# adam-kerrigan/pybader

Hardware: AMD Instinct MI355X
Metric: Mvoxels/s neargrid assign+refine on 512^3 grid (higher is better)
Workload: dtype f64; 1 GPU; 512^3 synthetic 8-Gaussian-atom cubic cell (BASELINE config 3), neargrid assign + neargrid edge refinement changed:2, density resident in HBM; method=neargrid, device_driven_slab_step=False, basins=8

## Files before the change

include/bader_hip.h:

```cpp
#ifndef BADER_HIP_H
#define BADER_HIP_H

#include <stdint.h>

#ifdef __cplusplus
extern "C" {
#endif

typedef struct xb_ctx xb_ctx;

enum { XB_OK = 0, XB_E_ARG = -1, XB_E_HIP = -2, XB_E_STATE = -3, XB_E_LIMIT = -4, XB_E_COMM = -5,
       XB_E_SHORT = -6  };

enum { XB_I8 = 1, XB_I16 = 2, XB_I32 = 4, XB_I64 = 8 };

enum { XB_METHOD_ONGRID = 0, XB_METHOD_NEARGRID = 1 };
enum { XB_REFINE_ALL = 0, XB_REFINE_CHANGED = 1 };

const char *xb_last_error(void);
int xb_device_count(void);
int xb_create(int device, xb_ctx **out);
void xb_destroy(xb_ctx *c);
int xb_sync(xb_ctx *c);
void *xb_stream(xb_ctx *c);
// ... 172 lines not shown
int xb_brick_masks(xb_ctx *c, void **dev_ptr, int64_t *n_bricks, int64_t *own_first, int64_t *own_count);
int xb_table_ties(xb_ctx *c, int64_t *has_ties);
int xb_table_finish(xb_ctx *c, const int64_t *seeds, int64_t n_seeds, int64_t any_ties);

void *xb_labels_ptr(xb_ctx *c);
void *xb_known_ptr(xb_ctx *c);
void *xb_density_ptr(xb_ctx *c);
int64_t xb_plane_elems(xb_ctx *c);
int xb_copy_planes(xb_ctx *c, int which , int to_device, void *host, int64_t xa, int64_t xb);
int xb_label_wire(xb_ctx *c, int widen_to, int *wire_out);
int xb_brick_masks_copy(xb_ctx *c, int to_device, int32_t *host, int64_t first, int64_t count);
int xb_set_halo(xb_ctx *c, int64_t halo);

int xb_slab_supported(xb_ctx *c, int nranks, int64_t *ok);
int xb_slab_assign_masks(xb_ctx *c, int rank, int nranks);
int xb_slab_assign_trace(xb_ctx *c);
int xb_slab_assign_finish(xb_ctx *c, int64_t *n_maxima, int64_t *status);
int xb_slab_refine_pass(xb_ctx *c);
int xb_slab_walkers_round(xb_ctx *c, int src, int last);
int xb_slab_walk_layout(xb_ctx *c, int64_t out[5]);
int xb_slab_walk_send(xb_ctx *c, int64_t walkers);
enum {
    XB_XC_EDGES = 0,
    XB_XC_CHANGED = 1,
    XB_XC_ESCAPED = 2,
    XB_XC_TRAVELLING = 3,
    XB_XC_SLOW = 4,
    XB_XC_LOST = 5,
    XB_XC_MINE = 6,
    XB_XC_ROUNDS = 7,
    XB_XC_COUNT = 8
};
int xb_slab_refine_counts(xb_ctx *c, int64_t *local, int64_t *global);
int xb_slab_block(xb_ctx *c, int which, void **dev_ptr, int64_t *bytes_total, int64_t *own_offset, int64_t *own_bytes);
int xb_slab_block_copy(xb_ctx *c, int which, int to_device, void *host, int64_t off, int64_t bytes);
int xb_host_waits(int64_t *n);

enum {
    XB_TIMER_ASSIGN = 0,
    XB_TIMER_OG_MASKS = 1,
    XB_TIMER_EDGE_FIND = 2,
    XB_TIMER_REFINE_TRACE = 3,
    XB_TIMER_MASKS_GROWTH = 4,
    XB_TIMER_BRICK_MASKS = 5,
    XB_TIMER_TRACE = 6,
    XB_TIMER_BRICK_RECORDS = 7,
    XB_TIMER_MOMENTS = 8,
    XB_TIMER_ADJACENCY = 9,
    XB_TIMER_MERGE = 10,
    XB_TIMER_COUNT = 11
};
int xb_kernel_time(xb_ctx *c, int which, double *ms_total, int64_t *launches);
int xb_kernel_time_reset(xb_ctx *c);
int xb_enable_timing(xb_ctx *c, int on);
enum {
    XB_OPT_REGIONS = 1,
    XB_OPT_CROSS_CHECK = 2,
    XB_OPT_DEBUG = 3,
    XB_OPT_EC_GROUPS = 4,
    XB_OPT_EC_QCAP = 5,
    XB_OPT_DROP_TABLE = 6,
    XB_OPT_KILL_LAUNCHES = 17,
    XB_OPT_SELF_EXCHANGE = 19,
    XB_OPT_ASYNC_COMM = 24,
    XB_OPT_WEIGHT_NO_LABELS = 30
};
enum {
    XB_REGIONS_BOXES = 1,
    XB_REGIONS_BRICKS = 2
};
enum { XB_DROP_TABLE_AND_MAXIMA = 2 };
enum {
    XB_CHECK_NO_MIRROR = 1,
    XB_CHECK_GENERIC_WALKER = 2,
    XB_CHECK_FULL_TGRAD = 4,
    XB_CHECK_LIST_DILATE = 8,
    XB_CHECK_WIDE_HALO = 16,
    XB_CHECK_NO_EC_SHARE = 32,
    XB_CHECK_IO_GATHER = 64
};
#define XB_CHECK_BRICK_LOOKUP 128
#define XB_CHECK_VOXEL_SWEEP 256
#define XB_CHECK_GENERIC_RETRACE 512
enum {
    XB_DBG_EC_PASSES = 4,
    XB_DBG_SLAB_STATS = 16,
    XB_DBG_STAGE_WAIT = 32,
    XB_DBG_SHORT_TIERS = 64
};
#define XB_DBG_KEEP_RETRACE_OVERFLOW 128
int xb_set_option(xb_ctx *c, int key, int value);
int xb_host_alloc(int64_t bytes, void **out);
int xb_host_free(void *p);
int xb_memory_stats(xb_ctx *c, int64_t *bytes_total, int64_t *bytes_table, int64_t *bytes_scratch);
int xb_box_stats(xb_ctx *c, int64_t *n_boxes, int64_t *box_voxels);
int xb_brick_labels(xb_ctx *c, int32_t *out, int64_t capacity, int64_t dims[3]);
int xb_slow_path_stats(xb_ctx *c, int64_t *assign_total, int64_t *refine_total);
int xb_deferred_stats(xb_ctx *c, int64_t *refine_total);
int xb_sweep_stats(xb_ctx *c, int64_t *bit_sweeps, int64_t *voxel_sweeps);
int xb_retrace_stats(xb_ctx *c, int64_t *lean_launches, int64_t *generic_launches);
int xb_trace_stats(xb_ctx *c, int64_t *nb_lean_launches, int64_t *lookup_lean_launches, int64_t *generic_launches,
                   int64_t *wide_lean_launches);
int xb_retrace_overflow(xb_ctx *c, int32_t *out, int64_t capacity, int64_t *n);
int xb_edge_list(xb_ctx *c, int32_t *out, int64_t capacity, int64_t *edges, int64_t *tiles_listed);
int xb_growth_stats(xb_ctx *c, int64_t *retries, int64_t *kill_launches);

int xb_comm_unique_id(uint8_t id_out[128]);
int xb_comm_init(xb_ctx *c, int rank, int nranks, const uint8_t id_in[128]);
int xb_comm_destroy(xb_ctx *c);
int xb_comm_exchange_planes(xb_ctx *c, int which, int n_send, const int32_t *send_peer, const int64_t *send_xa,
                            const int64_t *send_xb, int n_recv, const int32_t *recv_peer, const int64_t *recv_xa,
                            const int64_t *recv_xb);
int xb_comm_allreduce_i64(xb_ctx *c, int64_t *inout, int64_t n, int op);
int xb_comm_allgather_i64(xb_ctx *c, const int64_t *in, int64_t n, int64_t *out);
int xb_comm_share_brick_masks(xb_ctx *c, const int64_t *first, const int64_t *count);
int xb_comm_allgather_block(xb_ctx *c, int which, const int64_t *first, const int64_t *count);
int xb_comm_allreduce_block(xb_ctx *c);
int xb_comm_info(xb_ctx *c, int64_t out[4]);
int xb_comm_stats(xb_ctx *c, int64_t *bytes_sent);

#ifdef __cplusplus
}
#endif
#endif
```

pybader_amd/_lib.py:

```python
import ctypes as C
import threading
import os

import numpy as np

HERE = os.path.dirname(os.path.abspath(__file__))
LIB_PATH = os.environ.get('XB_LIBRARY') or os.path.join(HERE, 'libbader_hip.so')

METHODS = {'ongrid': 0, 'neargrid': 1}
REFINE_MODES = {'all': 0, 'changed': 1}
DTYPE_CODE = {np.dtype(np.int8): 1, np.dtype(np.int16): 2, np.dtype(np.int32): 4, np.dtype(np.int64): 8}
(XB_XC_EDGES, XB_XC_CHANGED, XB_XC_ESCAPED, XB_XC_TRAVELLING, XB_XC_SLOW, XB_XC_LOST, XB_XC_MINE, XB_XC_ROUNDS,
 XB_XC_COUNT) = range(9)
(XB_TIMER_ASSIGN, XB_TIMER_OG_MASKS, XB_TIMER_EDGE_FIND, XB_TIMER_REFINE_TRACE, XB_TIMER_MASKS_GROWTH, XB_TIMER_BRICK_MASKS,
 XB_TIMER_TRACE, XB_TIMER_BRICK_RECORDS, XB_TIMER_MOMENTS, XB_TIMER_ADJACENCY, XB_TIMER_MERGE, XB_TIMER_COUNT) = range(12)
XB_OPT_REGIONS = 1
XB_REGIONS_BOXES, XB_REGIONS_BRICKS = 1, 2
XB_OPT_CROSS_CHECK = 2
(XB_CHECK_NO_MIRROR, XB_CHECK_GENERIC_WALKER, XB_CHECK_FULL_TGRAD, XB_CHECK_LIST_DILATE, XB_CHECK_WIDE_HALO,
 XB_CHECK_NO_EC_SHARE, XB_CHECK_IO_GATHER) = (1, 2, 4, 8, 16, 32, 64)
CROSS_CHECK_BRICK_LOOKUP = 128
CROSS_CHECK_VOXEL_SWEEP = 256
CROSS_CHECK_GENERIC_RETRACE = 512
XB_OPT_DEBUG = 3
XB_DBG_EC_PASSES, XB_DBG_SLAB_STATS, XB_DBG_STAGE_WAIT, XB_DBG_SHORT_TIERS = 4, 16, 32, 64
DEBUG_KEEP_RETRACE_OVERFLOW = 128
XB_OPT_EC_GROUPS = 4
XB_OPT_EC_QCAP = 5
XB_OPT_DROP_TABLE = 6
XB_DROP_TABLE_AND_MAXIMA = 2
XB_OPT_KILL_LAUNCHES = 17
XB_OPT_SELF_EXCHANGE = 19
XB_OPT_ASYNC_COMM = 24
XB_OPT_WEIGHT_NO_LABELS = 30
XB_VORONOI_FULL_SEARCH = 1
XB_VORONOI_CAND_MAX = 512
XB_CRITICAL_FLOOD = 1
(XB_CRITICAL_MAXIMA, XB_CRITICAL_BOND_VOXELS, XB_CRITICAL_BOND_SUM, XB_CRITICAL_RING_VOXELS, XB_CRITICAL_RING_SUM,
 XB_CRITICAL_MINIMA, XB_CRITICAL_COUNTS) = range(7)
XB_CRITICAL_FULL = 0x3fff
XB_CRITICAL_LUT_SIZE = 16384
XB_STENCIL_GATHER = 1
XB_STENCIL_COEFFS = 51
XB_STENCIL_POINT_VALUES = 10
NCI_C = float.fromhex('0x1.8bfd4dd6882cbp+2')
XB_NCI_ATTRACTIVE, XB_NCI_VDW, XB_NCI_REPULSIVE, XB_NCI_CLASSES = range(4)
XB_NCI_HIST_LDS_BINS = 1024
XB_NCI_BINS_MAX = 1 << 24
XB_ISO_GATHER = 1
XB_ISO_TABLE_SIZE = 768
ISO_NCI_RAISED = 100.0
XB_DOMAINS_ABOVE = 0
XB_DOMAINS_BELOW = 1
XB_DOMAINS_NCI = 2
XB_DOMAINS_GLOBAL = 1
XB_DOMAINS_SHARES_LIST = 2
XB_DOMAINS_GATHER = 4
XB_DOMAINS_TIMES = 8
XB_DOMAINS_SHARE_CELLS = 1 << 24
XB_HIRSHFELD_FULL_SEARCH = 1
XB_HIRSHFELD_CAND_MAX = 256
XB_HIRSHFELD_PROMOLECULE, XB_HIRSHFELD_DEFORMATION = 0, 1
XB_ISA_DIRECT = 2
XB_ISA_ITERS_MAX = 64
XB_MBIS_DIRECT = 2
XB_MBIS_KEEP = 4
XB_MBIS_ITERS_MAX = 64
XB_MBIS_SHELLS_MAX = 8
XB_STOCKMOM_DIRECT = 2

_vp, _i64, _dbl, _int = C.c_void_p, C.c_int64, C.c_double, C.c_int
_pi64, _pdbl = C.POINTER(C.c_int64), C.POINTER(C.c_double)
SYMBOLS = {
    'xb_last_error': (C.c_char_p, []),
    'xb_device_count': (_int, []),
    'xb_create': (_int, [_int, C.POINTER(_vp)]),
    'xb_destroy': (None, [_vp]),
    'xb_sync': (_int, [_vp]),
    'xb_stream': (_vp, [_vp]),
    'xb_set_grid': (_int, [_vp, _pi64, _pdbl, _pdbl, _i64, _i64]),
    'xb_upload_density': (_int, [_vp, _vp]),
    'xb_synth_density': (_int, [_vp, _pdbl, _pdbl, _i64, _dbl]),
    'xb_parse_density_text': (_int, [_vp, _vp, _i64, _dbl, _pi64, _pi64]),
    'xb_parse_cube_text': (_int, [_vp, _vp, _i64, _i64, _i64, _int, _dbl, _pi64, _pi64]),
    'xb_download_density': (_int, [_vp, _vp]),
    'xb_format_begin': (_int, [_vp, _vp, _pi64, _int, _dbl, _int, _int, _vp, _i64, _i64, _pi64]),
    'xb_format_host_values': (_int, [_vp, _vp, _vp]),
    'xb_format_set_host_text': (_int, [_vp, _vp, _vp]),
    'xb_format_next': (_int, [_vp, C.POINTER(_vp), _pi64]),
    'xb_format_times': (_int, [_vp, _pdbl, _pdbl]),
    'xb_format_end': (_int, [_vp]),
    'xb_upload_labels': (_int, [_vp, _vp, _int]),
    'xb_download_labels': (_int, [_vp, _vp, _int]),
    'xb_import_density': (_int, [_vp, _vp, _int, _pi64, _vp]),
    'xb_import_labels': (_int, [_vp, _vp, _int, _vp]),
    'xb_export_labels': (_int, [_vp, _vp, _int, _vp]),
    'xb_export_volume': (_int, [_vp, _i64, _vp, _int, _vp]),
    'xb_device_alloc': (_int, [_int, _i64, C.POINTER(_vp)]),
    'xb_device_free': (_int, [_vp]),
    'xb_device_read': (_int, [_vp, _vp, _vp, _i64, _vp]),
    'xb_upload_known': (_int, [_vp, _vp]),
    'xb_download_known': (_int, [_vp, _vp]),
    'xb_vacuum_assign': (_int, [_vp, _dbl, _dbl, _pdbl, _pdbl]),
    'xb_assign': (_int, [_vp, _int, _pi64]),
    'xb_get_maxima': (_int, [_vp, _vp, _i64]),
    'xb_assign_trace': (_int, [_vp, _int, _pi64]),
# ... 24 lines not shown
    'xb_adjacency_release': (_int, [_vp]),
    'xb_merge_basins': (_int, [_vp, _vp, _int, _i64, _vp, _dbl, _i64, _pi64, _pi64, C.POINTER(_int)]),
    'xb_merge_fetch': (_int, [_vp, _vp, _vp, _vp, _i64]),
    'xb_merge_release': (_int, [_vp]),
    'xb_weight_sum': (_int, [_vp, _pdbl, _dbl, _vp, _pi64]),
    'xb_weight_sum_device': (_int, [_vp, _pdbl, _dbl, _vp, _int, _pi64, _vp, _pi64]),
    'xb_weight_fetch': (_int, [_vp, _vp, _vp, _vp, _i64]),
    'xb_weight_stats': (_int, [_vp, _pi64]),
    'xb_weight_release': (_int, [_vp]),
    'xb_voronoi_assign': (_int, [_vp, _pdbl, _pdbl, _i64, _dbl, _int, _pi64]),
    'xb_critical_lut': (_int, [_vp]),
    'xb_critical_points': (_int, [_vp, _dbl, _int, _pi64, _pi64]),
    'xb_critical_fetch': (_int, [_vp, _vp, _vp, _vp, _vp, _i64]),
    'xb_critical_bonds': (_int, [_vp, _i64, _pi64, _pi64]),
    'xb_critical_bonds_fetch': (_int, [_vp, _vp, _vp, _vp, _vp, _vp, _i64]),
    'xb_critical_release': (_int, [_vp]),
    'xb_stencil_coeffs': (_int, [_pdbl, _i64, _i64, _i64, _pdbl]),
    'xb_laplacian_field': (_int, [_vp, _pdbl, _int, _vp, _vp]),
    'xb_laplacian_sum': (_int, [_vp, _pdbl, _i64, _dbl, _int, _pdbl, _pdbl, _pdbl]),
    'xb_stencil_points': (_int, [_vp, _pdbl, _vp, _i64, _vp]),
    'xb_nci_field': (_int, [_vp, _pdbl, _int, _vp, _vp, _vp, _vp]),
    'xb_nci_sum': (_int, [_vp, _pdbl, _i64, _dbl, _dbl, _dbl, _dbl, _int, _pi64, _pdbl, _pdbl]),
    'xb_nci_hist': (_int, [_vp, _pdbl, _pdbl, _i64, _pdbl, _i64, _int, _pi64]),
    'xb_isosurface_table': (_int, [_vp]),
    'xb_isosurface': (_int, [_vp, _vp, _vp, _pdbl, _dbl, _i64, _int, _pi64]),
    'xb_isosurface_fetch': (_int, [_vp, _int, _vp, _vp, _vp, _vp, _vp, _i64, _i64, _pdbl, _pdbl, _i64]),
    'xb_isosurface_release': (_int, [_vp]),
    'xb_isosurface_nci_mask': (_int, [_vp, _vp, _dbl]),
    'xb_regions_label': (_int, [_vp, _int, _vp, _dbl, _pdbl, _dbl, _dbl, _int, _pi64]),
    'xb_regions_sums': (_int, [_vp, _dbl, _dbl, _pi64, _pi64, _pi64, _pdbl, _pdbl, _pi64, _pdbl, _pdbl, _i64]),
    'xb_regions_shares': (_int, [_vp, _i64, _int, _pi64]),
    'xb_regions_shares_fetch': (_int, [_vp, _vp, _vp, _pi64, _i64]),
    'xb_regions_fetch_map': (_int, [_vp, _int, _vp]),
    'xb_regions_times': (_int, [_vp, _pdbl]),
    'xb_regions_release': (_int, [_vp]),
    'xb_stream_wait': (_int, [_vp, _vp]),
    'xb_device_write': (_int, [_vp, _vp, _vp, _i64]),
    'xb_hirshfeld_images': (_int, [_pdbl, _pdbl, _vp, _i64, _pdbl, _i64, _pi64, _vp, _i64]),
    'xb_hirshfeld_setup': (_int, [_vp, _pdbl, _pdbl, _vp, _i64, _pdbl, _pdbl, _i64, _i64]),
    'xb_hirshfeld_release': (_int, [_vp]),
    'xb_hirshfeld_sum': (_int, [_vp, _dbl, _int, _pdbl, _pdbl, _pdbl, _pi64]),
    'xb_hirshfeld_field': (_int, [_vp, _int, _int, _vp, _vp]),
    'xb_isa_setup': (_int, [_vp, _pdbl, _pdbl, _i64, _pdbl, _i64, _pdbl, _dbl, _pi64]),
    'xb_isa_iterate': (_int, [_vp, _i64, _int, _pi64, _pi64]),
    'xb_isa_tables': (_int, [_vp, _pdbl, _pi64]),
    'xb_isa_load': (_int, [_vp, _pdbl]),
    'xb_isa_rho_bound': (_int, [_vp, _pdbl]),
    'xb_mbis_setup': (_int, [_vp, _pdbl, _pdbl, _i64, _pdbl, _vp, _pdbl, _i64, _i64, _pdbl, _pdbl, _dbl, _dbl, _pi64]),
    'xb_mbis_iterate': (_int, [_vp, _i64, _int, _pi64, _pi64, _pi64, _pi64]),
    'xb_mbis_params': (_int, [_vp, _pdbl, _pdbl, _pi64]),
    'xb_mbis_load': (_int, [_vp, _pdbl, _pdbl]),
    'xb_mbis_field': (_int, [_vp, _int, _int, _vp, _vp]),
    'xb_stockholder_moments': (_int, [_vp, _dbl, _int, _pi64, _pi64, _pi64]),
    'xb_volume_assign': (_int, [_vp, _vp, _i64]),
    'xb_atom_assign': (_int, [_vp, _i64, _vp, _i64, _vp, _vp, _vp]),
    'xb_surface_distance': (_int, [_vp, _vp, _vp, _i64, _vp, _pi64]),
    'xb_volume_mask': (_int, [_vp, _i64, _vp]),
    'xb_label_sum': (_int, [_vp, _i64, _pdbl, _pi64]),
    'xb_set_table_window': (_int, [_vp, _i64]),
    'xb_table_build': (_int, [_vp, _pi64]),
    'xb_table_local_seeds': (_int, [_vp, _vp, _i64]),
    'xb_brick_masks': (_int, [_vp, C.POINTER(_vp), _pi64, _pi64, _pi64]),
    'xb_table_ties': (_int, [_vp, _pi64]),
    'xb_table_finish': (_int, [_vp, _vp, _i64, _i64]),
    'xb_labels_ptr': (_vp, [_vp]),
    'xb_known_ptr': (_vp, [_vp]),
    'xb_density_ptr': (_vp, [_vp]),
    'xb_plane_elems': (_i64, [_vp]),
    'xb_copy_planes': (_int, [_vp, _int, _int, _vp, _i64, _i64]),
    'xb_label_wire': (_int, [_vp, _int, _vp]),
    'xb_host_alloc': (_int, [_i64, _vp]),
    'xb_host_free': (_int, [_vp]),
    'xb_brick_masks_copy': (_int, [_vp, _int, _vp, _i64, _i64]),
    'xb_set_halo': (_int, [_vp, _i64]),
    'xb_kernel_time': (_int, [_vp, _int, _pdbl, _pi64]),
    'xb_kernel_time_reset': (_int, [_vp]),
    'xb_enable_timing': (_int, [_vp, _int]),
    'xb_set_option': (_int, [_vp, _int, _int]),
    'xb_box_stats': (_int, [_vp, _pi64, _pi64]),
    'xb_brick_labels': (_int, [_vp, _vp, _i64, _pi64]),
    'xb_slow_path_stats': (_int, [_vp, _pi64, _pi64]),
    'xb_deferred_stats': (_int, [_vp, _pi64]),
    'xb_sweep_stats': (_int, [_vp, _pi64, _pi64]),
    'xb_edge_list': (_int, [_vp, _vp, _i64, _pi64, _pi64]),
    'xb_retrace_stats': (_int, [_vp, _pi64, _pi64]),
    'xb_trace_stats': (_int, [_vp, _pi64, _pi64, _pi64, _pi64]),
    'xb_axis_limits': (_int, [_vp, _pi64, _pi64]),
    'xb_retrace_overflow': (_int, [_vp, _vp, _i64, _pi64]),
    'xb_growth_stats': (_int, [_vp, _pi64, _pi64]),
    'xb_comm_unique_id': (_int, [_vp]),
    'xb_comm_init': (_int, [_vp, _int, _int, _vp]),
    'xb_comm_destroy': (_int, [_vp]),
    'xb_comm_exchange_planes': (_int, [_vp, _int, _int, _vp, _pi64, _pi64, _int, _vp, _pi64, _pi64]),
    'xb_comm_allreduce_i64': (_int, [_vp, _pi64, C.c_int64, _int]),
    'xb_comm_allgather_i64': (_int, [_vp, _pi64, C.c_int64, _pi64]),
    'xb_comm_share_brick_masks': (_int, [_vp, _pi64, _pi64]),
    'xb_comm_allgather_block': (_int, [_vp, _int, _pi64, _pi64]),
    'xb_comm_allreduce_block': (_int, [_vp]),
    'xb_slab_supported': (_int, [_vp, _int, _pi64]),
    'xb_slab_assign_masks': (_int, [_vp, _int, _int]),
    'xb_slab_assign_trace': (_int, [_vp]),
    'xb_slab_assign_finish': (_int, [_vp, _pi64, _pi64]),
    'xb_slab_refine_pass': (_int, [_vp]),
    'xb_slab_walkers_round': (_int, [_vp, _int, _int]),
    'xb_slab_walk_layout': (_int, [_vp, _pi64]),
    'xb_slab_walk_send': (_int, [_vp, _i64]),
    'xb_slab_refine_counts': (_int, [_vp, _pi64, _pi64]),
    'xb_slab_block': (_int, [_vp, _int, C.POINTER(_vp), _pi64, _pi64, _pi64]),
    'xb_slab_block_copy': (_int, [_vp, _int, _int, _vp, _i64, _i64]),
    'xb_host_waits': (_int, [_pi64]),
    'xb_comm_stats': (_int, [_vp, _pi64]),
    'xb_comm_info': (_int, [_vp, _pi64]),
    'xb_memory_stats': (_int, [_vp, _pi64, _pi64, _pi64]),
}

_lib = None


class BaderHipError(RuntimeError):
    code = None


XB_E_ARG = -1
XB_E_STATE = -3
XB_E_LIMIT = -4
XB_E_SHORT = -6


def load():
    global _lib
    if _lib is None:
        if not os.path.exists(LIB_PATH):
            raise BaderHipError(f"{LIB_PATH} is missing: build it with `python -m pybader_amd.build` "
                                "(hipcc, gfx950); pybader_amd has no CPU fallback")
        lib = C.CDLL(LIB_PATH)
        for name, (res, args) in SYMBOLS.items():
            fn = getattr(lib, name)
            fn.restype = res
            fn.argtypes = args
        _lib = lib
    return _lib


_POOL_KEEP = 4
_POOL_MAX_BYTES = 4 << 30


class _PinnedBuf:
    __slots__ = ('ptr', 'nbytes', '__weakref__')

    def __init__(self, ptr, nbytes):
        self.ptr, self.nbytes = ptr, nbytes

    @property
    def __array_interface__(self):
        return {'shape': (self.nbytes,), 'typestr': '|u1', 'data': (self.ptr, False), 'version': 3}


_pool = {}
_pool_bytes = 0
_pool_lock = threading.Lock()


def _host_free(ptr):
    if _lib is not None:
        _lib.xb_host_free(C.c_void_p(ptr))
# ... 1008 lines not shown
    def slab_block(self, which):
        p, a, b, d = _vp(), C.c_int64(0), C.c_int64(0), C.c_int64(0)
        check(self.lib.xb_slab_block(self.h, int(which), C.byref(p), C.byref(a), C.byref(b), C.byref(d)))
        return int(p.value or 0), int(a.value), int(b.value), int(d.value)

    def slab_block_copy(self, which, host, off, to_device):
        assert host.dtype == np.uint8 and host.flags.c_contiguous
        check(self.lib.xb_slab_block_copy(self.h, int(which), 1 if to_device else 0, _ptr(host), int(off), host.nbytes))

    def comm_allgather_block(self, which, first, count):
        f, n = np.array(first, np.int64), np.array(count, np.int64)
        check(self.lib.xb_comm_allgather_block(self.h, int(which), f.ctypes.data_as(_pi64), n.ctypes.data_as(_pi64)))

    def comm_allreduce_block(self):
        check(self.lib.xb_comm_allreduce_block(self.h))

    def host_waits(self):
        a = C.c_int64(0)
        check(self.lib.xb_host_waits(C.byref(a)))
        return int(a.value)

    def memory_stats(self):
        a, b, d = C.c_int64(0), C.c_int64(0), C.c_int64(0)
        check(self.lib.xb_memory_stats(self.h, C.byref(a), C.byref(b), C.byref(d)))
        return int(a.value), int(b.value), int(d.value)

    def comm_info(self):
        out = (C.c_int64 * 4)()
        check(self.lib.xb_comm_info(self.h, out))
        return {'nccl_comm_count': int(out[0]), 'nccl_user_rank': int(out[1]), 'nccl_device': int(out[2]), 'rccl_version': int(out[3])}

    def comm_bytes_sent(self):
        n = C.c_int64(0)
        check(self.lib.xb_comm_stats(self.h, C.byref(n)))
        return int(n.value)

    def enable_timing(self, on=True, only=None):
        mask = int(bool(on)) if only is None else sum(2 << int(k) for k in only)
        check(self.lib.xb_enable_timing(self.h, mask))

    def kernel_time(self, which):
        ms, n = C.c_double(), C.c_int64()
        check(self.lib.xb_kernel_time(self.h, int(which), C.byref(ms), C.byref(n)))
        return ms.value, n.value

    def kernel_time_reset(self):
        check(self.lib.xb_kernel_time_reset(self.h))

    def set_option(self, key, value):
        check(self.lib.xb_set_option(self.h, int(key), int(value)))

    def box_stats(self):
        a, b = C.c_int64(), C.c_int64()
        check(self.lib.xb_box_stats(self.h, C.byref(a), C.byref(b)))
        return a.value, b.value

    def brick_labels(self):
        dims = (C.c_int64 * 3)()
        check(self.lib.xb_brick_labels(self.h, None, 0, dims))
        out = np.zeros(tuple(int(d) for d in dims), np.int32)
        check(self.lib.xb_brick_labels(self.h, _ptr(out), out.size, dims))
        return out

    def slow_path_stats(self):
        a, b = C.c_int64(), C.c_int64()
        check(self.lib.xb_slow_path_stats(self.h, C.byref(a), C.byref(b)))
        return a.value, b.value

    def growth_stats(self):
        a, b = C.c_int64(), C.c_int64()
        check(self.lib.xb_growth_stats(self.h, C.byref(a), C.byref(b)))
        return a.value, b.value

    def deferred_stats(self):
        a = C.c_int64()
        check(self.lib.xb_deferred_stats(self.h, C.byref(a)))
        return a.value

    def sweep_stats(self):
        a, b = C.c_int64(), C.c_int64()
        check(self.lib.xb_sweep_stats(self.h, C.byref(a), C.byref(b)))
        return a.value, b.value

    def retrace_stats(self):
        a, b = C.c_int64(), C.c_int64()
        check(self.lib.xb_retrace_stats(self.h, C.byref(a), C.byref(b)))
        return a.value, b.value

    def trace_stats(self):
        a, b, g = C.c_int64(), C.c_int64(), C.c_int64()
        check(self.lib.xb_trace_stats(self.h, C.byref(a), C.byref(b), C.byref(g), None))
        return a.value, b.value, g.value

    def trace_offset_stats(self):
        a, b, w = C.c_int64(), C.c_int64(), C.c_int64()
        check(self.lib.xb_trace_stats(self.h, C.byref(a), C.byref(b), None, C.byref(w)))
        return a.value + b.value - w.value, w.value

    def axis_limits(self):
        a, b = C.c_int64(), C.c_int64()
        check(self.lib.xb_axis_limits(self.h, C.byref(a), C.byref(b)))
        return a.value, b.value

    def retrace_overflow(self):
        n = C.c_int64()
        check(self.lib.xb_retrace_overflow(self.h, None, 0, C.byref(n)))
        out = np.zeros(n.value, np.int32)
        if n.value:
            check(self.lib.xb_retrace_overflow(self.h, _ptr(out), out.size, C.byref(n)))
        return out

    def edge_list(self):
        n, t = C.c_int64(), C.c_int64()
        check(self.lib.xb_edge_list(self.h, None, 0, C.byref(n), C.byref(t)))
        out = np.zeros(n.value, np.int32)
        if n.value:
            check(self.lib.xb_edge_list(self.h, _ptr(out), out.size, C.byref(n), C.byref(t)))
        return out, t.value

    def sync(self):
        check(self.lib.xb_sync(self.h))


def critical_lut():
    out = np.zeros(XB_CRITICAL_LUT_SIZE, np.uint8)
    check(load().xb_critical_lut(_ptr(out)))
    return out


def isosurface_table():
    out = np.zeros(XB_ISO_TABLE_SIZE, np.uint8)
    check(load().xb_isosurface_table(_ptr(out)))
    return out.reshape(6, 16, 8)


def hirshfeld_images(lattice, atoms_cart, species, r_cut):
    lat, at = _f64(lattice).reshape(9), _f64(atoms_cart).reshape(-1, 3)
    sp, rc = np.ascontiguousarray(species, dtype=np.int32).reshape(-1), _f64(r_cut).reshape(-1)
    if sp.shape[0] != at.shape[0]:
        raise ValueError(f'hirshfeld_images: {sp.shape[0]} species for {at.shape[0]} atoms')
    lib, m = load(), C.c_int64()
    args = (lat.ctypes.data_as(_pdbl), at.ctypes.data_as(_pdbl), _ptr(sp), at.shape[0], rc.ctypes.data_as(_pdbl), rc.shape[0])
    check(lib.xb_hirshfeld_images(*args, C.byref(m), None, 0))
    out = np.zeros((int(m.value), 4), np.int32)
    check(lib.xb_hirshfeld_images(*args, C.byref(m), _ptr(out), out.shape[0]))
    return out


def stencil_coeffs(lattice, shape):
    lat = _f64(lattice).reshape(9)
    out = np.zeros(XB_STENCIL_COEFFS, np.float64)
    nx, ny, nz = (int(s) for s in shape)
    check(load().xb_stencil_coeffs(lat.ctypes.data_as(_pdbl), nx, ny, nz, out.ctypes.data_as(_pdbl)))
    return out[:9].reshape(3, 3), out[9:15], out[15:].reshape(6, 6)


def atom_assign(bader_max_cart, atoms_cart, lattice):
    lib = load()
    bm, at, lat = _f64(bader_max_cart).reshape(-1, 3), _f64(atoms_cart).reshape(-1, 3), _f64(lattice).reshape(9)
    a, d = np.zeros(bm.shape[0], np.int64), np.zeros(bm.shape[0], np.float64)
    check(lib.xb_atom_assign(_ptr(bm), bm.shape[0], _ptr(at), at.shape[0], _ptr(lat), _ptr(a), _ptr(d)))
    return a, d


_default_ctx = {}

# ... 10 lines not shown
```

pybader_amd/csrc/bader_hip.hip:

```cpp
#include "bader_kernels.h"
#include "../../include/bader_hip.h"
#include "ctx_state.h"
#include "ctx_buffers.h"

#include <algorithm>
#include <cmath>
#include <cstdarg>
#include <cstdio>
#include <cstring>
#include <locale.h>
#include <mutex>
#include <numeric>
#include <string>
#include <thread>
#include <vector>

static thread_local long long xb_waits = 0;
static inline hipError_t xb_counted_sync(hipStream_t s) { xb_waits++; return (hipStreamSynchronize)(s); }
#define hipStreamSynchronize(s) xb_counted_sync(s)

#include "k_common.h"
#include "k_masks.h"
#include "k_fused.h"
#include "k_trace.h"
#include "k_ongrid.h"
#include "k_edges.h"
#include "k_sums.h"
#include "k_text.h"
#include "k_format.h"
#include "k_interop.h"
#include "k_weight.h"
#include "k_cell.h"
#include "k_moments.h"
#include "k_adjacency.h"
#include "k_merge.h"
#include "k_voronoi.h"
#include "k_critical.h"
#include "k_stencil.h"
#include "k_nci.h"
#include "k_hirshfeld.h"
#include "k_isa.h"
#include "k_mbis.h"
#include "k_stockmom.h"
#include "k_isosurface.h"
#include "k_regions.h"

static thread_local std::string g_err;
static int fail(int code, const char *fmt, ...) {
    char buf[512];
    va_list ap;
    va_start(ap, fmt);
    vsnprintf(buf, sizeof buf, fmt, ap);
    va_end(ap);
    g_err = buf;
    return code;
}
#define XB_BIG_CHUNK ((size_t)16 << 20)
#define HIPCHK(x)                                                                                   \
    do {                                                                                            \
        hipError_t e_ = (x);                                                                        \
        if (e_ != hipSuccess) return fail(XB_E_HIP, "%s:%d %s: %s", __FILE__, __LINE__, #x, hipGetErrorString(e_)); \
    } while (0)

struct TimedKernel {
    std::vector<std::pair<hipEvent_t, hipEvent_t>> pending;
    double ms = 0.;
    long long launches = 0;
};

namespace xbcomm { struct State; }
struct xb_ctx : CtxState, CtxBuffers {
    int device = 0;
    xbcomm::State *comm = nullptr;
    struct FmtState *fmt = nullptr;
    hipStream_t stream = nullptr;
    Grid g{};
    bool has_grid = false;
    long long N = 0;
    int halo = 0;
    double *rho = nullptr;
    GradRec *grad = nullptr;
    long long grad_cap = 0;
    long long list_cap = 0;
    int *ec_buf = nullptr;
    long long ec_buf_cap = 0;
    double *dist_dev = nullptr;
    int *boxbuf = nullptr;
    int *box_max_tab = nullptr;
    int n_boxes = 0;
    long long box_voxels = 0;
    struct Options {
        int boxes = 1, bricks = 1;
        int mirror = 1;
        int lean = 1;
        int mask_diag = 1;
        int tile_dilate = 1;
        int narrow_halo = 1;
        int ec_share = 1;
        int nb_bits = 1;
        int bit_sweep = 1;
        int lean_retrace = 1;
        int io_tiled = 1;
        int dbg = 0;
        int ec_groups = 256;
        int ec_qcap = EC_Q;
        int self_exchange = 0;
        int async_comm = 0;
        bool weight_no_labels = false;
    } opt;
    int *ec_share = nullptr;
    std::vector<int64_t> esc_starts, esc_offsets, esc_vox;
    unsigned long long *ec_pend = nullptr;
    int8_t *ec_pflag = nullptr;
    std::vector<int8_t> esc_complete;
    double vac_tol = 0.;
    bool regions_pending = false;
    bool buni_halo_safe = false;
    bool regions_neargrid = false;
    int n_walk = 0;
    int *walk = nullptr;
    int table_margin = -1;
    bool table_prebuilt = false;
    int table_stage = 0;
    std::vector<int> window_seeds;
    bool window_ties = true;
    bool slab_sparse = false;
    int ec_local_n = 0;
    int walk_n_out = 0;
    void *walk_out_dev = nullptr;
    std::vector<int64_t> walk_host, res_host;
    int walk_n_res = 0;
    void *walk_in = nullptr, *walk_out2 = nullptr, *walk_res = nullptr;
    long long walk_cap = 0;
    long long stat_deferred = 0;
    long long stat_bit_sweeps = 0, stat_voxel_sweeps = 0;
    long long stat_ovf_assign = 0, stat_ovf_refine = 0;
    long long stat_lean_retraces = 0, stat_generic_retraces = 0;
    long long stat_nb_traces = 0, stat_lookup_traces = 0, stat_generic_traces = 0;
    long long stat_wide_traces = 0;
    int max_grid[3] = {0, 0, 0};
    std::vector<int> dbg_retrace_ovf;
    int *bres_last = nullptr;
    int *blab = nullptr;
    int nbk[3] = {0, 0, 0};
    bool brick_max_blanket = false;
    int grad_cover = 0;
    unsigned char *brick_rec = nullptr;
    unsigned long long *nb_tab = nullptr;
    void *xbuf = nullptr;
    int slab_rank = 0, slab_nranks = 0, slab_stage = 0;
    void *wbuf[2] = {nullptr, nullptr};
    void *wk_in = nullptr;
    int wbuf_ranks = 0, walk_last = -1, walk_round = 0, wcap = 0;
    int walk_send = 0;
    int grow_kill_launches = 6;
    long long stat_grow_retries = 0;
    bool defer_wait = false;
    bool pending_assign = false;
    int64_t pending_n_maxima = 0;
    int grad_rule = 0;
    int *labels = nullptr;
    int8_t *known = nullptr;
    int *first = nullptr;
    int *list = nullptr;
    int8_t *st = nullptr;
    void *stage = nullptr;
    size_t stage_bytes = 0;
    int *max_list = nullptr;
    int *max_aux = nullptr;
    int max_cap = 0;
    int *ovf_list = nullptr;
    int ovf_cap = 0;
    int *counters = nullptr;
    int *fs = nullptr;
    int *blab_buf = nullptr;
    long long blab_alloc = 0;
    static constexpr int trace_waves = 8192;
    unsigned long long *counters64 = nullptr;
    double *dsum = nullptr;
    int *host_ints = nullptr;
    char *big_pin[2] = {nullptr, nullptr};
    hipEvent_t big_ev[2] = {nullptr, nullptr};
    hipEvent_t io_ev = nullptr;
    char *pin = nullptr;
    size_t pin_bytes = 0;
    std::vector<int> maxima_sorted;
    std::vector<int> local_max, local_first;
    bool first_clean = false;
    int list_n = 0;
    bool tiles_listed = false;
    unsigned timing = 0;
    TimedKernel tk[XB_TIMER_COUNT];
    long long n_alloc = 0;
    bool thin = false;
    long long w_stat[6] = {0, 0, 0, 0, 0, 0};
    bool w_have = false;
    std::vector<int64_t> w_idx;
    std::vector<double> w_charge, w_volume;
    bool aj_have = false;
    int aj_dirs = 0;
    std::vector<int32_t> aj_a, aj_b;
    std::vector<int64_t> aj_facets, aj_sfacet;
    std::vector<double> aj_saddle;
    bool mg_have = false;
    std::vector<int32_t> mg_root, mg_round;
    std::vector<double> mg_pers;
    size_t cp_n = 0, cp_bond_voxels = 0;
    bool cb_have = false;
    std::vector<unsigned long long> cp_rec;
    std::vector<int32_t> cb_a, cb_b;
    std::vector<int64_t> cb_saddles, cb_voxel;
    std::vector<double> cb_rho;
    size_t hs_acc = 0;
    bool hs_have = false;
    int64_t hs_n = 0;
    int hs_cus = 0;
    HsGeom hs_geom{};
    bool hs_isa = false;
    size_t isa_x = 0, isa_pairs0 = 0;
    int isa_e = 0, isa_cur = 0;
    double isa_bound = 0.;
    bool hs_mbis = false;
    size_t mbis_x = 0;
    int mbis_M = 0, mbis_MS = 0, mbis_cur = 0, mbis_e[4] = {0, 0, 0, 0};
    int64_t mbis_J = 0, mbis_KE = 0;
// ... 64 lines not shown
        if (std::memcmp(&a, &b, sizeof a) != 0) return false;
        s.dsym[idx] = a;
    }
    return true;
}

static void mirror_prefilter(const Grid &g, int &mirror, double &mu_scale) {
    mirror = 0;
    double dmin = 0.;
    bool first = true;
    for (int i = 0; i < 27; i++)
        if (i != 0) { dmin = first ? g.dist[i] : std::min(dmin, g.dist[i]); first = false; }
    if (!(dmin > 0.) || !std::isfinite(dmin)) { mu_scale = 0.; return; }
    for (int ax = 0; ax < 3; ax++) {
        bool ok = true;
        for (int u = 0; u < 3 && ok; u++)
            for (int v = 0; v < 3 && ok; v++) {
                int ip[3], im[3];
                ip[ax] = 1; im[ax] = 2;
                ip[(ax + 1) % 3] = im[(ax + 1) % 3] = u;
                ip[(ax + 2) % 3] = im[(ax + 2) % 3] = v;
                const double a = g.dist[ip[0] * 9 + ip[1] * 3 + ip[2]], b = g.dist[im[0] * 9 + im[1] * 3 + im[2]];
                ok = std::memcmp(&a, &b, sizeof a) == 0;
            }
        if (ok) mirror |= 1 << ax;
    }
    mu_scale = std::ldexp(1. + 1. / dmin, -48);
}

struct ScopedTimer {
    xb_ctx *c;
    int which;
    hipEvent_t a = nullptr, b = nullptr;
    ScopedTimer(xb_ctx *c_, int w) : c(c_), which(w) {
        if ((c->timing >> which) & 1u) {
            hipEventCreate(&a);
            hipEventCreate(&b);
            hipEventRecord(a, c->stream);
        }
    }
    ~ScopedTimer() {
        if ((c->timing >> which) & 1u) {
            hipEventRecord(b, c->stream);
            c->tk[which].pending.push_back({a, b});
        }
    }
};

extern "C" {

const char *xb_last_error(void) { return g_err.c_str(); }

#include "host_context.h"
#include "host_stages.h"
#include "host_format.h"
#include "host_assign.h"
#include "host_refine.h"
#include "host_sums.h"
#include "host_slab_table.h"
#include "host_interop.h"
#include "host_weight.h"
#include "host_cell.h"
#include "host_moments.h"
#include "host_adjacency.h"
#include "host_merge.h"
#include "host_voronoi.h"
#include "host_critical.h"
#include "host_stencil.h"
#include "host_nci.h"
#include "host_hirshfeld.h"
#include "host_isa.h"
#include "host_mbis.h"
#include "host_stockmom.h"
#include "host_isosurface.h"
#include "host_regions.h"
#include "host_analyses.h"

int xb_set_option(xb_ctx *c, int key, int value) {
    if (!c) return fail(XB_E_ARG, "null ctx");
    bool ok = true;
    switch (key) {
    case XB_OPT_REGIONS: c->opt.boxes = (value & XB_REGIONS_BOXES) != 0; c->opt.bricks = (value & XB_REGIONS_BRICKS) != 0; break;
    case XB_OPT_CROSS_CHECK:
        if (!(ok = value >= 0 && value < 2 * XB_CHECK_GENERIC_RETRACE)) break;
        c->opt.mirror = !(value & XB_CHECK_NO_MIRROR);
        c->opt.lean = !(value & XB_CHECK_GENERIC_WALKER);
        c->opt.mask_diag = !(value & XB_CHECK_FULL_TGRAD);
        c->opt.tile_dilate = !(value & XB_CHECK_LIST_DILATE);
        c->opt.narrow_halo = !(value & XB_CHECK_WIDE_HALO);
        c->opt.ec_share = !(value & XB_CHECK_NO_EC_SHARE);
        c->opt.io_tiled = !(value & XB_CHECK_IO_GATHER);
        c->opt.nb_bits = !(value & XB_CHECK_BRICK_LOOKUP);
        c->opt.bit_sweep = !(value & XB_CHECK_VOXEL_SWEEP);
        c->opt.lean_retrace = !(value & XB_CHECK_GENERIC_RETRACE);
        break;
    case XB_OPT_DEBUG: c->opt.dbg = value; break;
    case XB_OPT_EC_GROUPS: if ((ok = value >= 1 && value <= 4096)) c->opt.ec_groups = value; break;
    case XB_OPT_EC_QCAP: if ((ok = value >= 2 && value <= EC_Q)) c->opt.ec_qcap = value; break;
    case XB_OPT_DROP_TABLE: if (value == XB_DROP_TABLE_AND_MAXIMA) drop_table_and_maxima(*c); else drop_table(*c); break;
    case XB_OPT_KILL_LAUNCHES: if ((ok = value >= 1)) c->grow_kill_launches = value; break;
    case XB_OPT_SELF_EXCHANGE: c->opt.self_exchange = value != 0; break;
    case XB_OPT_ASYNC_COMM: c->opt.async_comm = value != 0; break;
    case XB_OPT_WEIGHT_NO_LABELS: c->opt.weight_no_labels = value != 0; break;
    default: ok = false;
    }
    if (!ok) return fail(XB_E_ARG, "xb_set_option: unknown key %d", key);
    return XB_OK;
}
int xb_growth_stats(xb_ctx *c, int64_t *retries, int64_t *kill_launches) {
    if (!c) return fail(XB_E_ARG, "null ctx");
    if (retries) *retries = c->stat_grow_retries;
    if (kill_launches) *kill_launches = c->grow_kill_launches;
    return XB_OK;
}
int xb_deferred_stats(xb_ctx *c, int64_t *refine_total) {
    if (!c) return fail(XB_E_ARG, "null ctx");
    if (refine_total) *refine_total = c->stat_deferred;
    return XB_OK;
}
int xb_sweep_stats(xb_ctx *c, int64_t *bit_sweeps, int64_t *voxel_sweeps) {
    if (!c) return fail(XB_E_ARG, "null ctx");
    if (bit_sweeps) *bit_sweeps = c->stat_bit_sweeps;
    if (voxel_sweeps) *voxel_sweeps = c->stat_voxel_sweeps;
    return XB_OK;
}
int xb_retrace_stats(xb_ctx *c, int64_t *lean_launches, int64_t *generic_launches) {
    if (!c) return fail(XB_E_ARG, "null ctx");
    if (lean_launches) *lean_launches = c->stat_lean_retraces;
    if (generic_launches) *generic_launches = c->stat_generic_retraces;
    return XB_OK;
}
int xb_trace_stats(xb_ctx *c, int64_t *nb_lean_launches, int64_t *lookup_lean_launches, int64_t *generic_launches, int64_t *wide_lean_launches) {
    if (!c) return fail(XB_E_ARG, "null ctx");
    if (wide_lean_launches) *wide_lean_launches = c->stat_wide_traces;
    if (nb_lean_launches) *nb_lean_launches = c->stat_nb_traces;
    if (lookup_lean_launches) *lookup_lean_launches = c->stat_lookup_traces;
    if (generic_launches) *generic_launches = c->stat_generic_traces;
    return XB_OK;
}
int xb_retrace_overflow(xb_ctx *c, int32_t *out, int64_t capacity, int64_t *n) {
    if (!c || !n || capacity < 0 || (capacity > 0 && !out)) return fail(XB_E_ARG, "xb_retrace_overflow: null ctx / count, or a capacity without a buffer");
    *n = (int64_t)c->dbg_retrace_ovf.size();
    if (capacity >= *n) {
        std::copy(c->dbg_retrace_ovf.begin(), c->dbg_retrace_ovf.end(), out);
        c->dbg_retrace_ovf.clear();
    }
    return XB_OK;
}
int xb_slow_path_stats(xb_ctx *c, int64_t *assign_total, int64_t *refine_total) {
    if (!c) return fail(XB_E_ARG, "null ctx");
    if (assign_total) *assign_total = c->stat_ovf_assign;
    if (refine_total) *refine_total = c->stat_ovf_refine;
    return XB_OK;
}
int xb_memory_stats(xb_ctx *c, int64_t *bytes_total, int64_t *bytes_table, int64_t *bytes_scratch) {
    if (!c || !c->has_grid) return fail(XB_E_STATE, "xb_memory_stats: no grid");
    const long long N = c->N;
    const long long table = c->grad_cap * (long long)sizeof(GradRec);
    const long long scratch = c->list_cap * 4 + (long long)c->stage_bytes + c->ec_buf_cap * 4 + (c->ec_pend ? 8 * N + 16 : 0) +
                              (long long)buf_counted_bytes(*c) ;
    const long long fixed = 8 * N  + 4 * N  + (N + 16)  + 4 * N  + N  +
                            2LL * c->max_cap * 4 + (long long)c->ovf_cap * 4 + c->blab_alloc * 13 + (long long)c->walk_cap * 3 * 80 +
                            (1 << 22) ;
    if (bytes_total) *bytes_total = fixed + table + scratch;
    if (bytes_table) *bytes_table = table;
    if (bytes_scratch) *bytes_scratch = scratch;
    return XB_OK;
}
int xb_box_stats(xb_ctx *c, int64_t *n_boxes, int64_t *box_voxels) {
    if (!c) return fail(XB_E_ARG, "null ctx");
    if (n_boxes) *n_boxes = c->n_boxes;
    if (box_voxels) *box_voxels = c->box_voxels;
    return XB_OK;
}
int xb_brick_labels(xb_ctx *c, int32_t *out, int64_t capacity, int64_t dims[3]) {
    if (!c || !c->has_grid) return fail(XB_E_STATE, "xb_brick_labels: no grid");
    if (!c->blab) return fail(XB_E_STATE, "xb_brick_labels: no trapping regions on this context (no neargrid assignment yet)");
    const int64_t nbr = (int64_t)c->nbk[0] * c->nbk[1] * c->nbk[2];
    if (dims) { dims[0] = c->nbk[0]; dims[1] = c->nbk[1]; dims[2] = c->nbk[2]; }
    if (!out) return XB_OK;
    if (capacity < nbr) return fail(XB_E_ARG, "xb_brick_labels: capacity too small");
    HIPCHK(hipSetDevice(c->device));
    HIPCHK(hipMemcpyAsync(out, c->blab, nbr * sizeof(int), hipMemcpyDeviceToHost, c->stream));
    HIPCHK(hipStreamSynchronize(c->stream));
    return XB_OK;
}
#ifdef XB_DEBUG_COUNT
int xb_debug_steps(xb_ctx *c, int on, signed char *host_out) {
    static signed char *buf = nullptr;
    if (host_out && buf) {
        if (hipMemcpy(host_out, buf, (size_t)c->N, hipMemcpyDeviceToHost) != hipSuccess) return XB_E_HIP;
    }
    if (on && !buf && hipMalloc(&buf, (size_t)c->N) != hipSuccess) return XB_E_HIP;
    if (on && hipMemset(buf, 0, (size_t)c->N) != hipSuccess) return XB_E_HIP;
    signed char *p = on ? buf : nullptr;
    return hipMemcpyToSymbol(HIP_SYMBOL(xb_dbg_steps), &p, sizeof p) == hipSuccess ? XB_OK : XB_E_HIP;
}
int xb_debug_counts(unsigned long long *out, int reset) {
    hipDeviceSynchronize();
    if (out && hipMemcpyFromSymbol(out, HIP_SYMBOL(xb_dbg), sizeof(unsigned long long) * 65536) != hipSuccess) return XB_E_HIP;
    if (reset) {
        static unsigned long long z[65536];
        if (hipMemcpyToSymbol(HIP_SYMBOL(xb_dbg), z, sizeof z) != hipSuccess) return XB_E_HIP;
    }
    return XB_OK;
}
// ... 42 lines not shown
```

pybader_amd/csrc/host_assign.h:

```cpp

static GridL light(const Grid &g);

static int ensure_brick_bytes(xb_ctx *c, int nbr) {
    if (c->blab_alloc < nbr) {
        hipFree(c->blab_buf); c->blab_buf = nullptr; c->blab_alloc = 0; c->brick_rec = nullptr; c->nb_tab = nullptr; c->brick_max_valid = false;
        if (c->grad_cover) { c->grad_cover = 0; drop_table(*c); }
        const size_t rec_bytes = ((size_t)nbr + 16 + 7) & ~(size_t)7;
        HIPCHK(hipMalloc(&c->blab_buf, (size_t)nbr * sizeof(int) + rec_bytes + (size_t)nbr * sizeof(unsigned long long)));
        c->blab_alloc = nbr;
        c->brick_rec = reinterpret_cast<unsigned char *>(c->blab_buf + nbr);
        c->nb_tab = reinterpret_cast<unsigned long long *>(c->brick_rec + rec_bytes);
    }
    return XB_OK;
}

static int ensure_grad(xb_ctx *c, bool force, bool boxes, bool main_rule) {
    if (int rc = need_grad(c)) return rc;
    c->g.main_ties = main_rule ? 1 : 0;
    if (c->grad_valid && !force && (c->grad_rule == 2 || c->grad_rule == (main_rule ? 1 : 0))) return XB_OK;
    const Grid &g = c->g;
    if (c->grad_valid && !force && !boxes && c->grad_cover == 1 && c->brick_rec) {
        const int nb1r = (g.ny + BRK - 1) / BRK, nb2r = (g.nz + BRK - 1) / BRK, nbr = ((g.nx + BRK - 1) / BRK) * nb1r * nb2r;
        ScopedTimer t(c, XB_TIMER_MASKS_GROWTH);
        launch_brick_records(c, nullptr, nullptr, nbr, nb1r, nb2r);
        HIPCHK(hipGetLastError());
        c->grad_rule = main_rule ? 1 : 0;
        return XB_OK;
    }
    if (!force && !boxes && !table_windowed(c) && g.x0 == 0 && g.x1 == g.nx && g.nx >= 16 && g.ny >= 16 && g.nz >= 16) {
        const int nb0 = (g.nx + BRK - 1) / BRK, nb1 = (g.ny + BRK - 1) / BRK, nb2 = (g.nz + BRK - 1) / BRK, nbr = nb0 * nb1 * nb2;
        if (int rc = ensure_brick_bytes(c, nbr)) return rc;
        ScopedTimer t(c, XB_TIMER_MASKS_GROWTH);
        int *buni = reinterpret_cast<int *>(c->st);
        if (!c->buni_valid) k_label_uniform_list<<<4096, TPB, 0, c->stream>>>(light(g), c->labels, nb1, nb2, nullptr, nbr, nullptr, nullptr, buni, 0, nbr);
        c->buni_valid = true;
        k_buni3<<<(nbr + 255) / 256, 256, 0, c->stream>>>(nb0, nb1, nb2, buni, buni + nbr);
        k_flag_mixed_bricks<<<(nbr + 255) / 256, 256, 0, c->stream>>>(nbr, buni + nbr, c->brick_rec);
        launch_brick_records(c, nullptr, nullptr, nbr, nb1, nb2);
        HIPCHK(hipGetLastError());
        c->grad_valid = true;
        c->grad_cover = 1;
        c->brick_max_blanket = true;
        c->grad_rule = main_rule ? 1 : 0;
        c->regions_labels = false;
        c->blab = nullptr;
        c->table_stage = 0;
        return XB_OK;
    }
    {
        const int nb0 = (g.nx + BRK - 1) / BRK, nb1 = (g.ny + BRK - 1) / BRK, nb2 = (g.nz + BRK - 1) / BRK, nbr = nb0 * nb1 * nb2;
        if (int rc = ensure_brick_bytes(c, nbr)) return rc;
        ScopedTimer t(c, XB_TIMER_MASKS_GROWTH);
        ScopedTimer t_masks(c, XB_TIMER_BRICK_MASKS);
        const int wb0 = table_windowed(c) ? g.wx0 / BRK : 0, wnb = table_windowed(c) ? g.wlen / BRK : nb0;
        k_flag_window_bricks<<<(nbr + 255) / 256, 256, 0, c->stream>>>(nb0, nb1 * nb2, wb0, wnb, (unsigned char)3, c->brick_rec);
        launch_brick_records(c, nullptr, nullptr, nbr, nb1, nb2);
        HIPCHK(hipGetLastError());
    }
    c->grad_valid = true;
    c->grad_cover = 1;
    c->brick_max_blanket = true;
    c->grad_rule = main_rule ? 1 : 0;
    c->window_ties = true;
    c->n_boxes = 0;
    c->box_voxels = 0;
    c->blab = nullptr;
    c->regions_labels = false;
    c->window_seeds.clear();
    c->table_stage = 2;
    (void)boxes;
    return XB_OK;
}

static int upload_pinned(xb_ctx *c, void *dst, const void *src, size_t bytes, size_t slot = 0) {
    if (!bytes) return XB_OK;
    if (slot + bytes > c->pin_bytes) {
        HIPCHK(hipStreamSynchronize(c->stream));
        const size_t want = std::max<size_t>(2 * (slot + bytes), 1 << 20);
        char *p = nullptr;
        HIPCHK(hipHostMalloc(&p, want));
        if (c->pin && slot) memcpy(p, c->pin, slot);
        hipHostFree(c->pin);
        c->pin = p; c->pin_bytes = want;
    }
    memcpy(c->pin + slot, src, bytes);
    HIPCHK(hipMemcpyAsync(dst, c->pin + slot, bytes, hipMemcpyHostToDevice, c->stream));
    return XB_OK;
}
static int download_pinned(xb_ctx *c, void *dst, const void *src_dev, size_t bytes) {
    if (!bytes) return XB_OK;
    if (bytes > c->pin_bytes) {
        HIPCHK(hipStreamSynchronize(c->stream));
        hipHostFree(c->pin); c->pin = nullptr; c->pin_bytes = 0;
        const size_t want = std::max<size_t>(2 * bytes, 1 << 20);
        HIPCHK(hipHostMalloc(&c->pin, want));
        c->pin_bytes = want;
    }
    HIPCHK(hipMemcpyAsync(c->pin, src_dev, bytes, hipMemcpyDeviceToHost, c->stream));
    HIPCHK(hipStreamSynchronize(c->stream));
    memcpy(dst, c->pin, bytes);
    return XB_OK;
}

#define XB_MID_K 32
static int run_slow(xb_ctx *c, int n, int refine, int *max_count = nullptr, int *changed = nullptr, int *escaped = nullptr, const int *list_in = nullptr,
                    const int *n_dev = nullptr, bool stage_free = false) {
    if (!max_count) max_count = c->counters + CT_N_MAX;
    if (!changed) changed = c->counters + CT_CHANGED;
    if (!escaped) escaped = c->counters + CT_ESCAPED;
    if (n <= 0) return XB_OK;
    const size_t budget = (size_t)128 << 20;
    const int tiers[3] = {(c->opt.dbg & XB_DBG_SHORT_TIERS) ? 3 : 64, (c->opt.dbg & XB_DBG_SHORT_TIERS) ? 5 : 2048, (c->opt.dbg & XB_DBG_SHORT_TIERS) ? 8 : 1 << 15};
    const bool blind = (size_t)n * tiers[1] <= budget;
    const size_t have = std::max<size_t>(std::min<size_t>(budget, (size_t)n * tiers[0]), blind ? (size_t)n * tiers[1] : 0) + (size_t)(1 << 15) * 64;
    const size_t n_lists = 2 * (size_t)n + 8;
    DevBuf<int> path_buf, lists_buf;
    int *path = nullptr, *lists = nullptr;
// ... 170 lines not shown
                max_count_dev = c->counters + CT_N_MAX;
            }
            if (int rc = run_slow(c, novf, 0)) return rc;
        }
        c->g.main_ties = 0;
    } else if (method == XB_METHOD_ONGRID) {
        c->zero_outside[0] = -1;
        c->blab = nullptr;
        c->n_boxes = 0;
        c->box_voxels = 0;
        {
            ScopedTimer t(c, XB_TIMER_OG_MASKS);
            const int small = small_grid(g);
            const int nbr = ((g.nx + BRK - 1) / BRK) * ((g.ny + BRK - 1) / BRK) * ((g.nz + BRK - 1) / BRK);
            if (3LL * nbr > c->list_cap) return fail(XB_E_LIMIT, "xb_assign: scratch too small for the brick arrays of the pointer pass");
            dim3 grid((g.nz + GT_Z - 1) / GT_Z, (g.ny + GT_Y - 1) / GT_Y, (g.nx + GT_X - 1) / GT_X);
            int *bm = c->list, *bmv = c->list + nbr, *bpt = c->list + 2 * nbr;
            GridS gs;
            if (sym_grid(g, gs)) k_og_masks<GridS, true><<<grid, TPB, 0, c->stream>>>(gs, c->rho, c->labels, small, c->has_vacuum ? 1 : 0, bm, bmv, bpt);
            else k_og_masks<Grid, true><<<grid, TPB, 0, c->stream>>>(g, c->rho, c->labels, small, c->has_vacuum ? 1 : 0, bm, bmv, bpt);
        }
        HIPCHK(hipGetLastError());
        box_max = c->boxbuf + BB_REGMAX;
        for (int it = 0; it < 64; it++) {
            HIPCHK(hipMemsetAsync(c->counters + CT_OG_MOVED, 0, sizeof(int), c->stream));
            k_og_jump<<<nblocks(c->N), TPB, 0, c->stream>>>(g, c->labels, c->counters + CT_OG_MOVED);
            HIPCHK(hipGetLastError());
            int nd = 0;
            if (int rc = read_counter(c, CT_OG_MOVED, &nd)) return rc;
            if (!nd) break;
            if (it == 63) return fail(XB_E_LIMIT, "ongrid pointer jumping did not converge");
        }
        k_note_roots<<<nblocks(own), TPB, 0, c->stream>>>(g, c->labels, c->first, c->max_list, c->counters + CT_N_MAX, c->max_cap);
        HIPCHK(hipGetLastError());
    } else
        return fail(XB_E_ARG, "xb_assign: unknown method %d", method);
    int nmax = 0;
    HIPCHK(hipMemcpyAsync(c->host_ints, max_count_dev, sizeof(int), hipMemcpyDeviceToHost, c->stream));
    HIPCHK(hipStreamSynchronize(c->stream));
    nmax = c->host_ints[0];
    if (nmax > c->max_cap) return fail(XB_E_LIMIT, "%d maxima exceed the table capacity %d", nmax, c->max_cap);
    c->local_max.resize(nmax);
    c->local_first.resize(nmax);
    if (nmax) {
        k_gather_first<<<(nmax + 255) / 256, 256, 0, c->stream>>>(c->first, c->max_list, nmax, c->max_aux);
        HIPCHK(hipGetLastError());
        if (int rc = download_pinned(c, c->local_max.data(), c->max_list, nmax * sizeof(int))) return rc;
        if (int rc = download_pinned(c, c->local_first.data(), c->max_aux, nmax * sizeof(int))) return rc;
    }
    if (n_local) *n_local = nmax;
    return XB_OK;
}

int xb_assign_local_table(xb_ctx *c, int64_t *max_idx, int64_t *first_idx, int64_t capacity) {
    NEED_GRID("xb_assign_local_table");
    if ((int64_t)c->local_max.size() > capacity) return fail(XB_E_ARG, "xb_assign_local_table: capacity too small");
    for (size_t i = 0; i < c->local_max.size(); i++) { max_idx[i] = c->local_max[i]; first_idx[i] = c->local_first[i]; }
    return XB_OK;
}

int xb_assign_finish(xb_ctx *c, const int64_t *max_idx_sorted, int64_t n_global) {
    NEED_GRID("xb_assign_finish");
    if (n_global > c->max_cap) return fail(XB_E_LIMIT, "xb_assign_finish: too many maxima");
    c->maxima_sorted.resize(n_global);
    for (int64_t i = 0; i < n_global; i++) c->maxima_sorted[i] = (int)max_idx_sorted[i];
    c->label_wire = label_wire_for(n_global);
    const Grid &g = c->g;
    if (n_global) {
        if (int rc = upload_pinned(c, c->max_aux, c->maxima_sorted.data(), n_global * sizeof(int))) return rc;
        k_set_rank<<<(unsigned)((n_global + 255) / 256), 256, 0, c->stream>>>(c->first, c->max_aux, (int)n_global);
        HIPCHK(hipGetLastError());
    }
    drop_label_marks(*c);
    const bool regions = c->regions_pending && c->blab;
    int buni = BUNI_NONE;
    if (regions && g.x1 - g.x0 == g.nx)
        buni = BUNI_SCAN;
    else if (regions && !c->has_vacuum && g.nx % 8 == 0 && g.ny % 8 == 0 && g.nz % 8 == 0 && g.x0 % 8 == 0 && g.x1 % 8 == 0)
        buni = BUNI_MIXED;
    launch_relabel(c, nullptr, (int)n_global, regions, c->box_max_tab ? c->box_max_tab : c->boxbuf + BB_REGMAX, buni, nullptr);
    HIPCHK(hipGetLastError());
    if (buni != BUNI_NONE) {
        c->buni_valid = true;
        c->buni_halo_safe = buni == BUNI_MIXED;
    }
    c->regions_labels = regions && !c->has_vacuum && c->regions_neargrid;
    c->regions_pending = false;
    HIPCHK(hipStreamSynchronize(c->stream));
    c->first_clean = true;
    return XB_OK;
}


static bool fused_ok(const xb_ctx *c) {
    const Grid &g = c->g;
    return c->opt.boxes && c->opt.bricks && g.x0 == 0 && g.x1 == g.nx && !table_windowed(c) &&
           g.nx >= 16 && g.ny >= 16 && g.nz >= 16;
}
static int assign_neargrid_tail(xb_ctx *c, int64_t *n_maxima);

static int fused_numbering_launch(xb_ctx *c) {
    k_number_maxima<<<1, 1024, 0, c->stream>>>(c->fs, c->first, c->max_list, c->max_cap, c->max_aux, c->fs + FS_TOTAL);
    launch_relabel(c, c->fs, 0, c->regions_pending, c->box_max_tab, BUNI_SCAN, c->bres_last);
    HIPCHK(hipGetLastError());
    return XB_OK;
}
static int number_maxima_big(xb_ctx *c, int nmax) {
    const long long n_words = (c->N + 31) / 32, n_blocks = (n_words + 1023) / 1024;
    const size_t need = (size_t)(2 * n_words + n_blocks) * sizeof(int);
    DevBuf<int> own;
    int *scratch = (int *)c->stage;
    if (!c->stage || c->stage_bytes < need) {
        HIPCHK(own.alloc((size_t)(2 * n_words + n_blocks)));
        scratch = own.p;
    }
    unsigned *bits = reinterpret_cast<unsigned *>(scratch);
    int *wprefix = scratch + n_words, *bsum = scratch + 2 * n_words;
    HIPCHK(hipMemsetAsync(bits, 0, (size_t)n_words * sizeof(int), c->stream));
    k_rank_mark<<<(nmax + 255) / 256, 256, 0, c->stream>>>(c->first, c->max_list, nmax, bits);
    k_rank_scan<<<(unsigned)n_blocks, 1024, 0, c->stream>>>(bits, (int)n_words, wprefix, bsum);
    k_rank_blocks<<<1, 1024, 0, c->stream>>>(bsum, (int)n_blocks);
    k_rank_assign<<<(nmax + 255) / 256, 256, 0, c->stream>>>(c->first, c->max_list, nmax, bits, wprefix, bsum, c->max_aux, c->fs);
    HIPCHK(hipGetLastError());
    launch_relabel(c, c->fs, 0, c->regions_pending, c->box_max_tab, BUNI_SCAN, c->bres_last);
    HIPCHK(hipGetLastError());
    c->maxima_sorted.resize(nmax);
    HIPCHK(hipMemcpyAsync(c->maxima_sorted.data(), c->max_aux, (size_t)nmax * sizeof(int), hipMemcpyDeviceToHost, c->stream));
    HIPCHK(hipStreamSynchronize(c->stream));
    return XB_OK;
}

static int assign_neargrid_fused(xb_ctx *c, int64_t *n_maxima) {
    if (int rc = need_grad(c)) return rc;
    Grid &g = c->g;
    const int nb0 = (g.nx + BRK - 1) / BRK, nb1 = (g.ny + BRK - 1) / BRK, nb2 = (g.nz + BRK - 1) / BRK, nbr = nb0 * nb1 * nb2;
    const bool part = g.nx % BRK || g.ny % BRK || g.nz % BRK;
    if (int rc = ensure_brick_bytes(c, nbr)) return rc;
    int *fs = c->fs;
    int *seed = c->list, *bmask = c->list + nbr, *buf0 = c->list + 2 * nbr, *buf1 = c->list + 3 * nbr, *walk = c->list + 4 * nbr;
    int *box_max = c->boxbuf + BB_REGMAX, *box_first = c->boxbuf + BB_REGFIRST;
    int *bmaxv = walk;
    int *bpot = c->list + 5 * nbr;
    int *bres = nullptr;
    c->box_max_tab = box_max;
    auto stage_done = [&](const char *what) {
        if (c->opt.dbg & XB_DBG_STAGE_WAIT) {
            const hipError_t e = (hipStreamSynchronize)(c->stream);
            int h16[16] = {0};
            (void)hipMemcpy(h16, fs, sizeof h16, hipMemcpyDeviceToHost);
            fprintf(stderr, "[assign] %s: %s  seeds %d regions %d certain %d walk %d maxima %d ovf %d err %d\n", what, hipGetErrorString(e), h16[FS_N_SEEDS],
                    h16[FS_N_BOXES], h16[FS_N_CERTAIN], h16[FS_N_WALK], h16[FS_N_MAX], h16[FS_N_OVF], h16[FS_ERR]);
            fflush(stderr);
        }
    };
    if (int rc = begin_assignment(c, fs, FS_TOTAL, true)) return rc;
    g.main_ties = 1;
    const GridL gl = light(g);
    {
        ScopedTimer t_growth(c, XB_TIMER_MASKS_GROWTH);
        {
            ScopedTimer t_masks(c, XB_TIMER_BRICK_MASKS);
            launch_brick_masks(c, part, true, bmask, bmaxv, bpot);
        }
        stage_done("brick masks");
        c->grad_valid = true;
        c->grad_rule = 1;
        c->grad_cover = 1;
        launch_region_growth(c, nb0, nb1, nb2, bmask, bmaxv, bpot, seed, buf0, buf1, box_max, box_first, true);
        HIPCHK(hipGetLastError());
        stage_done("region growth");
    }
    c->blab = c->blab_buf;
    c->regions_neargrid = true;
    c->walk = walk;
    c->nbk[0] = nb0; c->nbk[1] = nb1; c->nbk[2] = nb2;
    const long long own = c->N;
    {
        ScopedTimer t_assign(c, XB_TIMER_ASSIGN);
        {
            const bool vac = c->has_vacuum && c->vac_by_tol;
            launch_walk_list(c, nb0, nb1, nb2, walk, vac ? bpot : nullptr, c->vac_tol);
        }
        {
            ScopedTimer t_records(c, XB_TIMER_BRICK_RECORDS);
            launch_brick_records(c, walk, fs + FS_N_WALK, nbr, nb1, nb2);
        }
        stage_done("walk list + records");
        if (c->has_vacuum)
            k_fill_certain<<<nblocks(own), TPB, 0, c->stream>>>(gl, c->blab, nb1, nb2, box_max, c->labels, c->first, c->max_list,
                                                                fs + FS_N_MAX, c->max_cap, fs + FS_GROW_RETRY);
        else {
            k_note_regions<<<1, XB_BOXES_MAX, 0, c->stream>>>(gl, nb1, nb2, fs, box_first, box_max, c->first, c->max_list, fs + FS_N_MAX, c->max_cap);
            c->regions_pending = true;
        }
        {
            ScopedTimer t_trace(c, XB_TIMER_TRACE);
            int *bres_buf = c->has_vacuum ? nullptr : c->list + 6 * nbr;
            if (launch_persistent_trace(c, true, part, box_max, walk, c->has_vacuum ? 1 : 0, bres_buf)) bres = bres_buf;
        }
        HIPCHK(hipGetLastError());
        stage_done("trace");
    }
    c->bres_last = bres;
    if (int rc = fused_numbering_launch(c)) return rc;
    stage_done("numbering + relabel");
    HIPCHK(hipMemcpyAsync(c->host_ints, fs, (FS_TOTAL + XB_SORT_MAX) * sizeof(int), hipMemcpyDeviceToHost, c->stream));
    if (c->defer_wait) {
        g.main_ties = 0;
        c->grad_rule = 2;
        c->regions_pending = false;
        c->buni_valid = !c->has_vacuum;
        c->regions_labels = !c->has_vacuum;
        c->pending_assign = true;
        return XB_OK;
    }
    HIPCHK(hipStreamSynchronize(c->stream));
    return assign_neargrid_tail(c, n_maxima);
}

static int assign_neargrid_tail(xb_ctx *c, int64_t *n_maxima) {
    Grid &g = c->g;
    int *fs = c->fs;
    const int nb1 = c->nbk[1], nb2 = c->nbk[2];
    int *walk = c->walk, *box_max = c->box_max_tab;
    const int *h = c->host_ints;
    g.main_ties = 0;
    const GridL gl = light(g);
    if (h[FS_GROW_RETRY]) {
        c->grow_kill_launches = 1 << 20;
        c->stat_grow_retries++;
        drop_table(*c);
        return assign_neargrid_fused(c, n_maxima);
    }
    if (h[FS_TIES] == 0) c->grad_rule = 2;
    c->n_boxes = h[FS_N_BOXES];
    c->box_voxels = (long long)h[FS_N_CERTAIN] * BRK * BRK * BRK;
    c->n_walk = h[FS_N_WALK];
    const int novf = h[FS_N_OVF];
    int nmax = h[FS_N_MAX];
    if (nmax > c->max_cap) return fail(XB_E_LIMIT, "%d maxima exceed the table capacity %d", nmax, c->max_cap);
    c->stat_ovf_assign += novf;
    const int *sorted = h[FS_SORT_OK] && novf == 0 ? h + FS_TOTAL : nullptr;
    if (novf > 0) {
        g.main_ties = 1;
        const GridL glt = light(g);
        const int maxsteps = trace_maxsteps(g);
        int *list2 = (int *)c->stage;
        const int cap2 = (int)std::min<size_t>(c->stage_bytes / sizeof(int), 0x7fffffffu);
        auto two_tiers = [&](int n_listed) -> int {
            c->host_ints[HI_UPLOAD] = n_listed;
            HIPCHK(hipMemcpyAsync(c->counters + CT_MID_LISTED, c->host_ints + HI_UPLOAD, sizeof(int), hipMemcpyHostToDevice, c->stream));
            HIPCHK(hipMemsetAsync(c->counters + CT_MID_LEFT, 0, sizeof(int), c->stream));
            k_ng_trace_list<XB_MID_K><<<512, TPB, 0, c->stream>>>(glt, c->grad, box_max, c->blab, nb1, nb2, c->ovf_list, c->counters + CT_MID_LISTED, c->labels, c->first,
                                                          c->max_list, fs + FS_N_MAX, c->max_cap, list2, c->counters + CT_MID_LEFT, cap2, maxsteps, c->rho, c->dist_dev,
                                                          c->has_vacuum ? 1 : 0);
            HIPCHK(hipGetLastError());
            if (c->opt.dbg & XB_DBG_EC_PASSES) {
                int m2 = 0;
                if (int rc2 = read_counter(c, CT_MID_LEFT, &m2)) return rc2;
                fprintf(stderr, "[assign] %d walkers listed, %d left for the exact slow kernel after the %d-voxel window\n", n_listed, m2, XB_MID_K);
            }
            if (n_listed > cap2) return fail(XB_E_LIMIT, "%d walkers for the exact slow path exceed its list (%d)", n_listed, cap2);
            return run_slow(c, n_listed, 0, fs + FS_N_MAX, nullptr, nullptr, list2, c->counters + CT_MID_LEFT, true);
        };
        int rc = two_tiers(std::min(novf, c->ovf_cap));
        for (int left = novf - c->ovf_cap; !rc && left > 0;) {
            HIPCHK(hipMemsetAsync(c->counters + CT_N_OVF, 0, sizeof(int), c->stream));
            k_list_unfinished<<<4096, TPB, 0, c->stream>>>(gl, walk, fs + FS_N_WALK, nb1, nb2, c->labels, c->ovf_list, c->counters + CT_N_OVF, c->ovf_cap);
            HIPCHK(hipGetLastError());
            int m = 0;
            if ((rc = read_counter(c, CT_N_OVF, &m))) break;
            if (m == 0) break;
            rc = two_tiers(std::min(m, c->ovf_cap));
            left = m - c->ovf_cap;
        }
        g.main_ties = 0;
        if (rc) return rc;
        HIPCHK(hipMemsetAsync(fs + FS_N_OVF, 0, sizeof(int), c->stream));
        if (int rc2 = fused_numbering_launch(c)) return rc2;
        HIPCHK(hipMemcpyAsync(c->host_ints, fs, (FS_TOTAL + XB_SORT_MAX) * sizeof(int), hipMemcpyDeviceToHost, c->stream));
        HIPCHK(hipStreamSynchronize(c->stream));
        nmax = h[FS_N_MAX];
        if (nmax > c->max_cap) return fail(XB_E_LIMIT, "%d maxima exceed the table capacity %d", nmax, c->max_cap);
        if (h[FS_SORT_OK]) sorted = h + FS_TOTAL;
    }
    if (!sorted) {
        if (int rc = number_maxima_big(c, nmax)) return rc;
    }
    numbering_done(c, sorted, nmax, n_maxima);
    c->buni_valid = !c->has_vacuum;
    c->regions_labels = !c->has_vacuum;
    return XB_OK;
}


static bool assign_neargrid_complete(xb_ctx *c, int64_t *n_maxima) {
    c->pending_assign = false;
    const int *h = c->host_ints;
    const int nmax = h[FS_N_MAX];
    if (h[FS_GROW_RETRY] || h[FS_TIES] != 0 || h[FS_N_OVF] != 0 || !h[FS_SORT_OK] || nmax > c->max_cap || nmax > XB_SORT_MAX) return false;
    c->n_boxes = h[FS_N_BOXES];
    c->box_voxels = (long long)h[FS_N_CERTAIN] * BRK * BRK * BRK;
    c->n_walk = h[FS_N_WALK];
    numbering_done(c, h + FS_TOTAL, nmax, n_maxima);
    return true;
}

static int assign_ongrid_fused(xb_ctx *c, int64_t *n_maxima) {
    Grid &g = c->g;
    const int nb0 = (g.nx + BRK - 1) / BRK, nb1 = (g.ny + BRK - 1) / BRK, nb2 = (g.nz + BRK - 1) / BRK, nbr = nb0 * nb1 * nb2;
    const bool part = g.nx % BRK || g.ny % BRK || g.nz % BRK;
    if (int rc = ensure_brick_bytes(c, nbr)) return rc;
    int *fs = c->fs;
    int *seed = c->list, *bmask = c->list + nbr, *buf0 = c->list + 2 * nbr, *buf1 = c->list + 3 * nbr, *walk = c->list + 4 * nbr;
    int *bmaxv = walk, *bpot = c->list + 5 * nbr;
    int *box_max = c->boxbuf + BB_REGMAX, *box_first = c->boxbuf + BB_REGFIRST;
    c->box_max_tab = box_max;
    if (int rc = begin_assignment(c, fs, FS_TOTAL, true)) return rc;
    c->zero_outside[0] = -1;
    const GridL gl = light(g);
    {
        ScopedTimer t(c, XB_TIMER_OG_MASKS);
        const int small = small_grid(g);
        dim3 grid((g.nz + GT_Z - 1) / GT_Z, (g.ny + GT_Y - 1) / GT_Y, (g.nx + GT_X - 1) / GT_X);
        GridS gs;
        if (sym_grid(g, gs)) {
            if (part) k_og_masks<GridS, true><<<grid, TPB, 0, c->stream>>>(gs, c->rho, c->labels, small, 0, bmask, bmaxv, bpot);
            else k_og_masks<GridS, false><<<grid, TPB, 0, c->stream>>>(gs, c->rho, c->labels, small, 0, bmask, bmaxv, bpot);
        } else {
            if (part) k_og_masks<Grid, true><<<grid, TPB, 0, c->stream>>>(g, c->rho, c->labels, small, 0, bmask, bmaxv, bpot);
            else k_og_masks<Grid, false><<<grid, TPB, 0, c->stream>>>(g, c->rho, c->labels, small, 0, bmask, bmaxv, bpot);
        }
    }
    {
        ScopedTimer t_growth(c, XB_TIMER_MASKS_GROWTH);
        launch_region_growth(c, nb0, nb1, nb2, bmask, bmaxv, bpot, seed, buf0, buf1, box_max, box_first, true);
        HIPCHK(hipGetLastError());
    }
    drop_table(*c);
    c->grad_cover = 0;
    c->brick_max_valid = true;
    c->brick_max_blanket = false;
    c->blab = c->blab_buf;
    c->regions_neargrid = false;
    c->walk = walk;
    c->bres_last = nullptr;
    c->nbk[0] = nb0; c->nbk[1] = nb1; c->nbk[2] = nb2;
    {
        ScopedTimer t_assign(c, XB_TIMER_ASSIGN);
        launch_walk_list(c, nb0, nb1, nb2, walk, nullptr, 0.);
        k_note_regions<<<1, XB_BOXES_MAX, 0, c->stream>>>(gl, nb1, nb2, fs, box_first, box_max, c->first, c->max_list, fs + FS_N_MAX, c->max_cap);
        c->regions_pending = true;
        k_og_walk_dev<<<16384, XB_WAVE, 0, c->stream>>>(gl, box_max, c->blab, nb1, nb2, walk, fs, c->labels, c->first, c->max_list, c->max_cap,
                                                        1 << 22);
        HIPCHK(hipGetLastError());
    }
    if (int rc = fused_numbering_launch(c)) return rc;
    HIPCHK(hipMemcpyAsync(c->host_ints, fs, (FS_TOTAL + XB_SORT_MAX) * sizeof(int), hipMemcpyDeviceToHost, c->stream));
    HIPCHK(hipStreamSynchronize(c->stream));
    const int *h = c->host_ints;
    if (h[FS_GROW_RETRY]) {
        c->grow_kill_launches = 1 << 20;
        c->stat_grow_retries++;
        return assign_ongrid_fused(c, n_maxima);
    }
    if (h[FS_ERR] & 1) return fail(XB_E_STATE, "ongrid pointer chase did not terminate");
    c->n_boxes = h[FS_N_BOXES];
    c->box_voxels = (long long)h[FS_N_CERTAIN] * BRK * BRK * BRK;
    c->n_walk = h[FS_N_WALK];
    const int nmax = h[FS_N_MAX];
    if (nmax > c->max_cap) return fail(XB_E_LIMIT, "%d maxima exceed the table capacity %d", nmax, c->max_cap);
    const int *sorted = h[FS_SORT_OK] ? h + FS_TOTAL : nullptr;
    if (!sorted) {
        if (int rc = number_maxima_big(c, nmax)) return rc;
    }
    numbering_done(c, sorted, nmax, n_maxima);
    c->buni_valid = true;
    return XB_OK;
}

static int sort_and_finish(xb_ctx *c, int64_t n, int64_t *n_maxima);
int xb_assign(xb_ctx *c, int method, int64_t *n_maxima) {
    NEED_GRID_RAW("xb_assign");
    c->have_labels = true;
    if (method == XB_METHOD_NEARGRID && fused_ok(c)) {
        if (c->has_vacuum) { if (int rc = settle_labels(c)) return rc; }
        else c->labels_zero_pending = false;
        return assign_neargrid_fused(c, n_maxima);
    }
    if (method == XB_METHOD_ONGRID && !c->has_vacuum) c->labels_zero_pending = false;
    if (method == XB_METHOD_ONGRID && !c->has_vacuum && fused_ok(c)) return assign_ongrid_fused(c, n_maxima);
    int64_t n = 0;
    if (int rc = xb_assign_trace(c, method, &n)) return rc;
    return sort_and_finish(c, n, n_maxima);
}
static int sort_and_finish(xb_ctx *c, int64_t n, int64_t *n_maxima) {
    std::vector<int> order(n);
    for (int i = 0; i < n; i++) order[i] = i;
    if (n <= 4096)
        std::sort(order.begin(), order.end(), [&](int a, int b) { return c->local_first[a] < c->local_first[b]; });
    else {
        std::vector<unsigned long long> a(n), b(n);
        for (int64_t i = 0; i < n; i++) a[i] = ((unsigned long long)(unsigned)c->local_first[i] << 32) | (unsigned)i;
        for (int pass = 0; pass < 3; pass++) {
            const int shift = 32 + 11 * pass;
            std::vector<int64_t> cnt(2049, 0);
            for (int64_t i = 0; i < n; i++) cnt[((a[i] >> shift) & 2047) + 1]++;
            for (int k = 0; k < 2048; k++) cnt[k + 1] += cnt[k];
            for (int64_t i = 0; i < n; i++) b[cnt[(a[i] >> shift) & 2047]++] = a[i];
            a.swap(b);
        }
        for (int64_t i = 0; i < n; i++) order[i] = (int)(a[i] & 0xffffffffu);
    }
    std::vector<int64_t> sorted(n);
    for (int i = 0; i < n; i++) sorted[i] = c->local_max[order[i]];
    if (int rc = xb_assign_finish(c, sorted.data(), n)) return rc;
    if (n_maxima) *n_maxima = n;
    return XB_OK;
}

int xb_get_maxima(xb_ctx *c, int64_t *maxima_out, int64_t capacity) {
    NEED_GRID("xb_get_maxima");
    if ((int64_t)c->maxima_sorted.size() > capacity) return fail(XB_E_ARG, "xb_get_maxima: capacity too small");
    const Grid &g = c->g;
    for (size_t i = 0; i < c->maxima_sorted.size(); i++) {
        const int m = c->maxima_sorted[i];
        const int x = m / g.nyz, r = m - x * g.nyz;
        maxima_out[3 * i] = x; maxima_out[3 * i + 1] = r / g.nz; maxima_out[3 * i + 2] = r % g.nz;
    }
    return XB_OK;
}
```

pybader_amd/csrc/host_refine.h:

```cpp

static void plane_range(const Grid &g, int ext, int &xa, int &np) {
    const int own = g.x1 - g.x0;
    if (own + 2 * ext >= g.nx) { xa = 0; np = g.nx; }
    else { xa = ((g.x0 - ext) % g.nx + g.nx) % g.nx; np = own + 2 * ext; }
}

static int preset_known_planes(xb_ctx *c, int p0, int np) {
    const Grid &g = c->g;
    const int run1 = std::min(np, g.nx - p0);
    HIPCHK(hipMemsetAsync(c->known + (size_t)p0 * g.nyz, 2, (size_t)run1 * g.nyz, c->stream));
    if (np > run1) HIPCHK(hipMemsetAsync(c->known, 2, (size_t)(np - run1) * g.nyz, c->stream));
    return XB_OK;
}
static int *launch_brick_uniformity(xb_ctx *c, const GridL &gl, int b_off, int count, unsigned scan_grid) {
    const Grid &g = c->g;
    const int nb0 = (g.nx + 7) / 8, nb1 = (g.ny + 7) / 8, nb2 = (g.nz + 7) / 8, nbr = nb0 * nb1 * nb2;
    int *buni = reinterpret_cast<int *>(c->st);
    if (!c->buni_valid)
        k_label_uniform_list<<<scan_grid, TPB, 0, c->stream>>>(gl, c->labels, nb1, nb2, nullptr, count, nullptr, nullptr, buni, b_off, nbr);
    k_buni3<<<(nbr + 255) / 256, 256, 0, c->stream>>>(nb0, nb1, nb2, buni, buni + nbr);
    return buni + nbr;
}

static bool sweep_bits_ok(const xb_ctx *c, const int *buni) {
    const Grid &g = c->g;
    if (c->grad_valid && c->grad_cover == 1 && c->brick_max_blanket) return false;
    const long long nbr = (long long)((g.nx + 7) / 8) * ((g.ny + 7) / 8) * ((g.nz + 7) / 8);
    if (8 * (long long)c->maxima_sorted.size() >= nbr) return false;
    return c->opt.bit_sweep && c->opt.tile_dilate && buni && !c->has_vacuum && g.x0 == 0 && g.x1 == g.nx && g.nx % ET_X == 0 &&
           g.ny % ET_Y == 0 && g.nz % ET_Z == 0 && !small_grid(g);
}
static void launch_sweep_bits(xb_ctx *c, const GridL &gl, int ntiles, int *edge_count, const GradRec *G, const unsigned char *brec,
                              const int *tiles, const int *n_tiles) {
    k_edge_sweep_bits<<<std::min(ntiles, 2048), TPB, 0, c->stream>>>(gl, c->rho, c->labels, c->known, c->list, edge_count, G, brec, tiles, n_tiles);
    c->stat_bit_sweeps++;
}

static int edge_find_launch(xb_ctx *c, bool *dilate_owned) {
    const Grid &g = c->g;
    const bool whole = (g.x1 - g.x0 == g.nx);
    if (!whole && c->halo < 2) return fail(XB_E_STATE, "xb_edge_find: slab needs a label halo (xb_set_halo)");
    int xa, np, xb_, npd;
    const bool all = whole || (g.x1 - g.x0) + 2 * c->halo >= g.nx;
    plane_range(g, all ? g.nx : c->halo - 1, xa, np);
    plane_range(g, all ? g.nx : c->halo - 2, xb_, npd);
    HIPCHK(hipMemsetAsync(c->counters + CT_N_EDGES, 0, sizeof(int), c->stream));
    c->tiles_listed = false;
    {
        ScopedTimer t(c, XB_TIMER_EDGE_FIND);
        const GridL gl = light(g);
        const int small = small_grid(g);
        int *buni = nullptr;
        if ((g.nx % 8 == 0 && g.ny % 8 == 0 && g.nz % 8 == 0) || (whole && g.nx >= 16 && g.ny >= 16 && g.nz >= 16)) {
            const int per_plane = ((g.ny + 7) / 8) * ((g.nz + 7) / 8);
            int b_off = 0, count = ((g.nx + 7) / 8) * per_plane;
            if (!all && np + 32 < g.nx) {
                const int p0 = ((xa - 8) % g.nx + g.nx) % g.nx;
                b_off = (p0 / 8) * per_plane;
                count = ((np + 8 + 7 + (p0 % 8)) / 8 + 1) * per_plane;
            }
            if (!c->buni_valid) c->buni_halo_safe = false;
            buni = launch_brick_uniformity(c, gl, b_off, count, (unsigned)std::min(4096, (count + 3) / 4));
        }
        const GradRec *G = c->grad_valid ? c->grad : nullptr;
        const unsigned char *brec = c->grad_valid && c->grad_cover == 1 ? c->brick_rec : nullptr;
        if (whole && sweep_bits_ok(c, buni)) {
            const int ntiles = (g.nz / ET_Z) * (g.ny / ET_Y) * (g.nx / ET_X);
            int *tiles = (int *)c->stage;
            HIPCHK(hipMemsetAsync(c->known, 2, (size_t)c->N, c->stream));
            HIPCHK(hipMemsetAsync(c->counters + CT_TILES_OWN, 0, sizeof(int), c->stream));
            k_edge_tile_list<<<(ntiles + TPB - 1) / TPB, TPB, 0, c->stream>>>(gl, buni, tiles, c->counters + CT_TILES_OWN, 0, g.nx / ET_X);
            launch_sweep_bits(c, gl, ntiles, c->counters + CT_N_EDGES, G, brec, tiles, c->counters + CT_TILES_OWN);
            HIPCHK(hipGetLastError());
            c->tiles_listed = true;
            *dilate_owned = false;
            return XB_OK;
        }
        c->stat_voxel_sweeps++;
        if (whole || all) {
            dim3 grid((g.nz + ET_Z - 1) / ET_Z, (g.ny + ET_Y - 1) / ET_Y, (np + ET_X - 1) / ET_X);
            k_edge_flag_tiled<<<grid, TPB, 0, c->stream>>>(gl, c->rho, c->labels, c->known, xa, np, c->list,
                                                           c->counters + CT_N_EDGES, small, buni, G, brec, c->has_vacuum ? 0 : 1);
            if (!whole)
                k_edge_dilate<<<nblocks((long long)npd * g.nyz), TPB, 0, c->stream>>>(g, c->known, xb_, npd, -2);
        } else if (buni && g.x0 % ET_X == 0 && g.x1 % ET_X == 0 && g.ny % ET_Y == 0 &&
                   (g.x1 - g.x0) + 2 * ((c->halo - 1 + ET_X - 1) / ET_X * ET_X) <= g.nx) {
            const int own = g.x1 - g.x0, side4 = (c->halo - 1 + ET_X - 1) / ET_X * ET_X;
            const int nty = g.ny / ET_Y, ntz = (g.nz + ET_Z - 1) / ET_Z;
            const int left0 = ((g.x0 - side4) % g.nx + g.nx) % g.nx, right0 = g.x1 % g.nx;
            if (int rc = preset_known_planes(c, left0, side4 + own + side4)) return rc;
            const int n_own = (own / ET_X) * nty * ntz, n_halo = 2 * (side4 / ET_X) * nty * ntz;
            int *tiles_own = (int *)c->stage, *tiles_halo = tiles_own + n_own, *halo_list = tiles_halo + n_halo;
            HIPCHK(hipMemsetAsync(c->counters + CT_HALO_EDGES, 0, sizeof(int), c->stream));
            HIPCHK(hipMemsetAsync(c->counters + CT_TILES_OWN, 0, CT_INTS(CT_TILES_OWN, CT_TILES_HALO) * sizeof(int), c->stream));
            GridL ga = gl;
            ga.x0 = 0; ga.x1 = g.nx;
            k_edge_tile_list<<<(n_own + TPB - 1) / TPB, TPB, 0, c->stream>>>(gl, buni, tiles_own, c->counters + CT_TILES_OWN, g.x0 / ET_X, own / ET_X);
            k_edge_tile_list<<<(n_halo / 2 + TPB - 1) / TPB, TPB, 0, c->stream>>>(gl, buni, tiles_halo, c->counters + CT_TILES_HALO, left0 / ET_X, side4 / ET_X);
            k_edge_tile_list<<<(n_halo / 2 + TPB - 1) / TPB, TPB, 0, c->stream>>>(gl, buni, tiles_halo, c->counters + CT_TILES_HALO, right0 / ET_X, side4 / ET_X);
            k_edge_flag_listed<<<std::min(n_own, 2048), TPB, 0, c->stream>>>(gl, c->rho, c->labels, c->known, c->list, c->counters + CT_N_EDGES, small, G, brec,
                                                            c->has_vacuum ? 0 : 1, tiles_own, c->counters + CT_TILES_OWN);
            k_edge_flag_listed<<<std::min(n_halo, 2048), TPB, 0, c->stream>>>(ga, c->rho, c->labels, c->known, halo_list, c->counters + CT_HALO_EDGES, small, G, brec,
                                                             c->has_vacuum ? 0 : 1, tiles_halo, c->counters + CT_TILES_HALO);
            k_edge_dilate_list<<<2048, TPB, 0, c->stream>>>(gl, c->known, halo_list, 0, c->counters + CT_HALO_EDGES);
        } else {
            const int own = g.x1 - g.x0, side = c->halo - 1;
            int *halo_list = (int *)c->stage;
            HIPCHK(hipMemsetAsync(c->counters + CT_HALO_EDGES, 0, sizeof(int), c->stream));
            GridL ga = gl;
            ga.x0 = 0; ga.x1 = g.nx;
            dim3 grid((g.nz + ET_Z - 1) / ET_Z, (g.ny + ET_Y - 1) / ET_Y, (own + ET_X - 1) / ET_X);
            k_edge_flag_tiled<<<grid, TPB, 0, c->stream>>>(gl, c->rho, c->labels, c->known, g.x0, own, c->list,
                                                           c->counters + CT_N_EDGES, small, buni, G, brec, c->has_vacuum ? 0 : 1);
            grid.z = (side + ET_X - 1) / ET_X;
            k_edge_flag_tiled<<<grid, TPB, 0, c->stream>>>(ga, c->rho, c->labels, c->known, xa, side, halo_list,
                                                           c->counters + CT_HALO_EDGES, small, buni, G, brec, c->has_vacuum ? 0 : 1);
            k_edge_flag_tiled<<<grid, TPB, 0, c->stream>>>(ga, c->rho, c->labels, c->known, g.x1 % g.nx, side, halo_list,
                                                           c->counters + CT_HALO_EDGES, small, buni, G, brec, c->has_vacuum ? 0 : 1);
            k_edge_dilate_list<<<2048, TPB, 0, c->stream>>>(gl, c->known, halo_list, 0, c->counters + CT_HALO_EDGES);
        }
    }
    HIPCHK(hipGetLastError());
    *dilate_owned = whole || !all;
    return XB_OK;
}
int xb_edge_find(xb_ctx *c, int64_t *edges) {
    NEED_GRID("xb_edge_find");
    const Grid &g = c->g;
    bool dilate_owned = false;
    stage_clobbered(*c);
    if (int rc = edge_find_launch(c, &dilate_owned)) return rc;
    int n = 0;
    if (int rc = read_counter(c, CT_N_EDGES, &n)) return rc;
    if (dilate_owned && n) {
        ScopedTimer t(c, XB_TIMER_EDGE_FIND);
        k_edge_dilate_list<<<nblocks(n), TPB, 0, c->stream>>>(light(g), c->known, c->list, n, nullptr);
        HIPCHK(hipGetLastError());
    }
    c->list_n = n;
    c->list_valid = true;
    if (edges) *edges = (int64_t)n;
    return XB_OK;
}

int xb_edge_list(xb_ctx *c, int32_t *out, int64_t capacity, int64_t *edges, int64_t *tiles_listed) {
    NEED_GRID("xb_edge_list");
    if (!c->list_valid) return fail(XB_E_STATE, "xb_edge_list: call xb_edge_find first (its list is gone once `known` is rewritten)");
    if (edges) *edges = c->list_n;
    if (tiles_listed) {
// ... 424 lines not shown
        if (n) {
            HIPCHK(hipMemcpyAsync(c->list, (int *)c->stage + c->N, (size_t)n * sizeof(int), hipMemcpyDeviceToDevice, c->stream));
            HIPCHK(hipMemcpyAsync(c->host_ints + HI_EC_CHGLIST, c->fs + FS_N_CHGLIST, sizeof(int), hipMemcpyDeviceToHost, c->stream));
            listed = true;
        }
    } else if (int rc = compact(c, -2, &n)) return rc;
    if (int rc = edge_check_resolve(c, n, nullptr, 0, g.nx, 0, c->N, checked, edges)) return rc;
    if (listed && c->host_ints[HI_EC_CHGLIST] != n) return fail(XB_E_STATE, "xb_edge_check: %d voxels listed for %d relabelled ones", c->host_ints[HI_EC_CHGLIST], n);
    return XB_OK;
}

int xb_edge_check_local(xb_ctx *c, int64_t *n_out) {
    NEED_GRID("xb_edge_check_local");
    drop_edge_lists(*c);
    int n = 0;
    if (int rc = compact(c, -2, &n)) return rc;
    if (n) {
        k_ec_class<<<nblocks(n), TPB, 0, c->stream>>>(c->g, c->rho, c->labels, c->list, n, c->st);
        HIPCHK(hipGetLastError());
    }
    c->ec_local_n = n;
    if (n_out) *n_out = n;
    return XB_OK;
}
int xb_edge_check_local_fetch(xb_ctx *c, int64_t *idx_out, int8_t *cls_out) {
    NEED_GRID("xb_edge_check_local_fetch");
    const int n = c->ec_local_n;
    if (!n) return XB_OK;
    std::vector<int> tmp(n);
    HIPCHK(hipMemcpyAsync(tmp.data(), c->list, n * sizeof(int), hipMemcpyDeviceToHost, c->stream));
    HIPCHK(hipMemcpyAsync(cls_out, c->st, n, hipMemcpyDeviceToHost, c->stream));
    HIPCHK(hipStreamSynchronize(c->stream));
    for (int i = 0; i < n; i++) idx_out[i] = tmp[i];
    return XB_OK;
}
int xb_edge_check_global(xb_ctx *c, const int64_t *idx, const int8_t *cls, int64_t n, int64_t *checked, int64_t *edges) {
    NEED_GRID("xb_edge_check_global");
    const Grid &g = c->g;
    drop_edge_lists(*c); c->buni_valid = false;
    if (checked) *checked = 0;
    if (edges) *edges = 0;
    if (n < 0 || n > c->N) return fail(XB_E_ARG, "xb_edge_check_global: bad list length");
    if (c->halo < 3 && g.vlen < g.nx) return fail(XB_E_STATE, "xb_edge_check_global: needs a halo of at least 3 planes");
    if (!n) return XB_OK;
    std::vector<int> i32(n);
    for (int64_t k = 0; k < n; k++) {
        if (idx[k] < 0 || idx[k] >= c->N) return fail(XB_E_ARG, "xb_edge_check_global: voxel index out of range");
        i32[k] = (int)idx[k];
    }
    if (g.vlen < g.nx)
        if (int rc = preset_known_planes(c, (g.vx0 + g.vlen) % g.nx, g.nx - g.vlen)) return rc;
    int8_t *dcls = c->st + (c->N - n);
    if (2 * n > c->N || 2 * n > c->list_cap) return fail(XB_E_LIMIT, "xb_edge_check_global: list longer than half the grid / the list buffer");
    if (int rc = upload_pinned(c, c->list, i32.data(), n * sizeof(int))) return rc;
    if (int rc = upload_pinned(c, dcls, cls, n, (n * sizeof(int) + 255) & ~(size_t)255)) return rc;
    k_scatter_byte<<<(unsigned)((n + 255) / 256), 256, 0, c->stream>>>(c->known, c->list, (int)n, (int8_t)-2);
    HIPCHK(hipGetLastError());
    int near_xa = 0, near_np = g.nx;
    if (g.vlen + 4 < g.nx) { near_xa = (g.vx0 - 2 + g.nx) % g.nx; near_np = g.vlen + 4; }
    const int rc = edge_check_resolve(c, (int)n, dcls, near_xa, near_np, (long long)g.x0 * g.nyz, (long long)g.x1 * g.nyz, checked, edges);
    return rc;
}

int xb_prepare_refine(xb_ctx *c) {
    NEED_GRID("xb_prepare_refine");
    return ensure_grad(c, false, false, false);
}

#define XB_STEP_REDO 1000
static int refine_iteration_fused(xb_ctx *c, int64_t *edges, int64_t *changed, bool late_records = false) {
    const Grid &g = c->g;
    int *fs = c->fs;
    c->g.main_ties = 0;
    const GridL gl = light(g);
    static_assert(FS_N_CHGLIST == FS_N_EDGES + 6, "one memset clears the refinement's counters");
    HIPCHK(hipMemsetAsync(fs + FS_N_EDGES, 0, 7 * sizeof(int), c->stream));
    stage_clobbered(*c);
    bool bits = false;
    {
        ScopedTimer t(c, XB_TIMER_EDGE_FIND);
        const int small = small_grid(g);
        int *buni = nullptr;
        int ntiles_listed = 0;
        if (g.nx >= 16 && g.ny >= 16 && g.nz >= 16)
            buni = launch_brick_uniformity(c, gl, 0, ((g.nx + 7) / 8) * ((g.ny + 7) / 8) * ((g.nz + 7) / 8), 4096);
        const unsigned char *brec = (c->grad_valid && c->grad_cover == 1) || late_records ? c->brick_rec : nullptr;
        if (buni) {
            const int ntiles = ((g.nz + ET_Z - 1) / ET_Z) * ((g.ny + ET_Y - 1) / ET_Y) * ((g.nx + ET_X - 1) / ET_X);
            ntiles_listed = ntiles;
            int *tiles = (int *)c->stage;
            HIPCHK(hipMemsetAsync(c->known, 2, (size_t)c->N, c->stream));
            k_edge_tile_list<<<(ntiles + TPB - 1) / TPB, TPB, 0, c->stream>>>(gl, buni, tiles, fs + FS_N_TILES, 0, (g.nx + ET_X - 1) / ET_X,
                                                                              c->pending_assign ? fs : nullptr);
            if ((bits = sweep_bits_ok(c, buni)))
                launch_sweep_bits(c, gl, ntiles, fs + FS_N_EDGES, c->grad_valid ? c->grad : nullptr, brec, tiles, fs + FS_N_TILES);
            else
                k_edge_flag_listed<<<std::min(ntiles, 2048), TPB, 0, c->stream>>>(gl, c->rho, c->labels, c->known, c->list, fs + FS_N_EDGES, small,
                                                               c->grad_valid ? c->grad : nullptr, brec, c->has_vacuum ? 0 : 1, tiles, fs + FS_N_TILES);
        } else {
            dim3 grid((g.nz + ET_Z - 1) / ET_Z, (g.ny + ET_Y - 1) / ET_Y, (g.nx + ET_X - 1) / ET_X);
            k_edge_flag_tiled<<<grid, TPB, 0, c->stream>>>(gl, c->rho, c->labels, c->known, 0, g.nx, c->list, fs + FS_N_EDGES, small, buni,
                                                           c->grad_valid ? c->grad : nullptr, brec, c->has_vacuum ? 0 : 1);
        }
        if (!bits) {
            if (buni && c->opt.tile_dilate && g.nz % ET_Z == 0) k_edge_dilate_tiles<<<std::min(ntiles_listed, 4096), TPB, 0, c->stream>>>(gl, c->known, (const int *)c->stage, fs + FS_N_TILES);
            else k_edge_dilate_list<<<nblocks(c->N / 16), TPB, 0, c->stream>>>(gl, c->known, c->list, 0, fs + FS_N_EDGES);
        }
    }
    if (!bits) c->stat_voxel_sweeps++;
    drop_edge_lists(*c); c->buni_valid = false;
    if (late_records) {
        if (int rc = need_grad(c)) return rc;
        ScopedTimer t(c, XB_TIMER_MASKS_GROWTH);
        const int nb0 = (g.nx + 7) / 8, nb1 = (g.ny + 7) / 8, nb2 = (g.nz + 7) / 8, nbr = nb0 * nb1 * nb2;
        unsigned char *band = reinterpret_cast<unsigned char *>(c->blab_buf);
        HIPCHK(hipMemsetAsync(band, 0, (size_t)nbr, c->stream));
        k_flag_band_bricks<<<4096, TPB, 0, c->stream>>>(gl, c->known, (const int *)c->stage, fs + FS_N_TILES, band);
        k_rec_set_bit0<<<(nbr + 255) / 256, 256, 0, c->stream>>>(nbr, c->brick_rec, band);
        launch_brick_records(c, nullptr, nullptr, nbr, nb1, nb2);
        HIPCHK(hipGetLastError());
        c->grad_valid = true;
        c->grad_cover = 1;
        c->grad_rule = 0;
        drop_label_marks(*c);
        c->blab = nullptr;
        c->table_stage = 0;
    }
    const unsigned char *brec = c->grad_cover == 1 ? c->brick_rec : nullptr;
    const int regions_ok = c->grad_cover == 1 && c->regions_labels && !c->has_vacuum ? 1 : 0;
    {
        ScopedTimer t(c, XB_TIMER_REFINE_TRACE);
        int *defer = (int *)c->stage;
        WalkerIO wl{};
        constexpr int XB_RT_BLOCK = 128;
        launch_edge_retrace(c, (unsigned)((c->N / 16 + XB_RT_BLOCK - 1) / XB_RT_BLOCK), XB_RT_BLOCK, c->list, 0, fs + FS_N_EDGES, fs + FS_CHANGED,
                            fs + FS_ESCAPED, fs + FS_R_OVF, brec, false, defer, fs + FS_R_DEFER, regions_ok, nullptr);
        if (c->grad_cover == 1 && !regions_ok)
            launch_refine_trace<2, true>(c, 512, TPB, (int *)c->stage, 0, fs + FS_R_DEFER, fs + FS_CHANGED, fs + FS_ESCAPED, c->ovf_list,
                                         fs + FS_R_OVF, c->ovf_cap, c->brick_rec, nullptr, nullptr, 0, nullptr, wl);
    }
    HIPCHK(hipGetLastError());
    int *hr = c->host_ints + HI_REFINE;
    HIPCHK(hipMemcpyAsync(hr, fs + FS_N_EDGES, 7 * sizeof(int), hipMemcpyDeviceToHost, c->stream));
    HIPCHK(hipStreamSynchronize(c->stream));
    if (c->pending_assign && !assign_neargrid_complete(c, &c->pending_n_maxima)) return XB_STEP_REDO;
    *edges = hr[0];
    *changed = hr[1];
    const int novf = hr[3];
    if (novf == 0 && hr[1] > 0 && c->stage_bytes >= 8 * (size_t)c->N && hr[1] <= (int)std::min<long long>(c->N, 0x7fffffffLL)) {
        k_list_changed<<<1024, TPB, 0, c->stream>>>(c->list, fs + FS_N_EDGES, c->known, (int *)c->stage + c->N, fs + FS_N_CHGLIST,
                                                    (int)std::min<long long>(c->N, 0x7fffffffLL), fs + FS_CHANGED);
        HIPCHK(hipGetLastError());
        c->chg_n = hr[1];
    } else if (novf == 0 && hr[1] == 0)
        c->chg_n = 0;
    c->stat_deferred += hr[4];
    if (hr[2]) return fail(XB_E_STATE, "xb_refine: %d traces left the grid", hr[2]);
    if (novf > c->ovf_cap) return fail(XB_E_LIMIT, "%d retraces need the slow path (cap %d)", novf, c->ovf_cap);
    c->stat_ovf_refine += novf;
    if (int rc = keep_retrace_overflow(c, novf)) return rc;
    if (novf > 0) {
        const int *slow_list = nullptr, *slow_n_dev = nullptr;
        const int n_slow = novf;
        const bool can_defer = c->grad_cover == 1 && !regions_ok;
        if (!can_defer && c->stage_bytes >= sizeof(int) * (size_t)novf) {
            int *list2 = (int *)c->stage;
            HIPCHK(hipMemsetAsync(c->counters + CT_MID_LEFT, 0, sizeof(int), c->stream));
            launch_refine_trace<XB_MID_K, false>(c, nblocks(novf), TPB, c->ovf_list, novf, nullptr, fs + FS_CHANGED, fs + FS_ESCAPED, list2,
// ... 111 lines not shown
```

pybader_amd/csrc/host_stages.h:

```cpp

enum { BB_TOTAL = 1 << 20, BB_REGMAX = 1 << 16, BB_REGFIRST = 1 << 17 };

static bool table_windowed(const xb_ctx *c) { return c->g.wlen < c->g.nx; }
static int small_grid(const Grid &g) { return g.nx < 16 || g.ny < 16 || g.nz < 80; }
static int trace_maxsteps(const Grid &g) { return 8 * (g.nx + g.ny + g.nz) + 64; }
static const int *slab_regions_of(const xb_ctx *c) {
    const Grid &g = c->g;
    return (table_windowed(c) && c->blab && c->regions_labels && !c->has_vacuum && (c->grad_rule == 2 || c->slab_sparse) &&
            g.nx % 8 == 0 && g.ny % 8 == 0 && g.nz % 8 == 0) ? c->blab : nullptr;
}

static_assert(CT_REDO == CT_N_MAX + 15, "a host-driven assignment zeroes CT_N_MAX .. CT_REDO at once");
static int begin_assignment(xb_ctx *c, int *counts, int n, bool invalidate) {
    HIPCHK(hipMemsetAsync(counts, 0, n * sizeof(int), c->stream));
    if (!c->first_clean) {
        k_fill<int><<<4096, TPB, 0, c->stream>>>(c->first, XB_INT_MAX, c->N);
        HIPCHK(hipGetLastError());
    }
    c->first_clean = false;
    c->regions_pending = false;
    if (invalidate) { drop_label_marks(*c); drop_edge_lists(*c); }
    return XB_OK;
}

static void launch_brick_masks(xb_ctx *c, bool part, bool allow_diag, int *bmask, int *bmaxv, int *bpot) {
    const Grid &g = c->g;
    const dim3 grid((g.nz + GT_Z - 1) / GT_Z, (g.ny + GT_Y - 1) / GT_Y, (g.x1 - g.x0 + GT_X - 1) / GT_X);
    GridS gs;
    const bool sym = sym_grid(g, gs);
    int mirror = 0;
    double mu_scale = 0.;
    if (sym && c->opt.mirror) mirror_prefilter(g, mirror, mu_scale);
    const bool diag = allow_diag && c->opt.mask_diag && g.T[1] == 0. && g.T[2] == 0. && g.T[3] == 0. && g.T[5] == 0. && g.T[6] == 0. && g.T[7] == 0.;
    auto launch = [&](auto kernel, const auto &gt) {
        kernel<<<grid, TPB, 0, c->stream>>>(gt, c->rho, small_grid(g), bmask, bmaxv, c->fs + FS_TIES, g.x0, mu_scale, mirror, bpot);
    };
    if (!sym) launch(part ? k_brick_masks<Grid, 1, false, true> : k_brick_masks<Grid, 1, false>, g);
    else if (part) launch(diag ? k_brick_masks<GridS, 1, true, true> : k_brick_masks<GridS, 1, false, true>, gs);
    else launch(diag ? k_brick_masks<GridS, 1, true> : k_brick_masks<GridS, 1, false>, gs);
    c->brick_max_blanket = false;
}

static bool nb_bits_ok(const xb_ctx *c) { return c->grad_valid && c->grad_nb && c->opt.nb_bits; }
static void launch_brick_records(xb_ctx *c, const int *list, const int *n_dev, int nbr, int nb1, int nb2) {
    const Grid &g = c->g;
    const bool part = g.nx % BRK || g.ny % BRK || g.nz % BRK;
    const bool mark = !table_windowed(c) && g.x0 == 0 && g.x1 == g.nx && !part && (!list || c->blab) && c->nb_tab;
    c->grad_nb = mark;
    if (mark)
        k_nb_table<<<(nbr + 255) / 256, 256, 0, c->stream>>>(nbr / (nb1 * nb2), nb1, nb2, list ? c->blab : nullptr, c->brick_rec, c->nb_tab);
    auto launch = [&](auto kernel, const auto &gt) {
        kernel<<<4096, TPB, 0, c->stream>>>(gt, c->rho, c->grad, list, n_dev, nbr, nb1, nb2, c->brick_rec, small_grid(g),
                                            mark ? c->nb_tab : nullptr);
    };
    GridS gs;
    if (sym_grid(g, gs)) launch(k_brick_records<GridS>, gs);
    else launch(k_brick_records<Grid>, g);
}

static void launch_region_growth(xb_ctx *c, int nb0, int nb1, int nb2, int *bmask, int *bmaxv, int *bpot, int *seed, int *buf0,
                                 int *buf1, int *box_max, int *box_first, bool chase) {
    const int nbr = nb0 * nb1 * nb2;
    int *fs = c->fs;
    k_seed_bricks<<<(nbr + 255) / 256, 256, 0, c->stream>>>(nbr, bmask, bmaxv, fs, seed, buf0, box_max, box_first);
    if (chase) {
        k_grow_parent<<<(nbr + TPB - 1) / TPB, TPB, 0, c->stream>>>(nb0, nb1, nb2, bmask, bpot, seed, buf1);
        k_grow_chase<<<(nbr + TPB - 1) / TPB, TPB, 0, c->stream>>>(nbr, buf1, seed, buf0, 4 * (nb0 + nb1 + nb2) + 64, fs);
    } else
        k_seed_finish<<<1, 1, 0, c->stream>>>(fs);
    const int long_schedule = 2 * ((std::max(std::max(nb0, nb1), nb2) + BG - 1) / BG) + 12;
    const int launches = chase ? std::min(long_schedule, c->grow_kill_launches) : long_schedule;
    const dim3 ggrid((nb2 + BG - 1) / BG, (nb1 + BG - 1) / BG, (nb0 + BG - 1) / BG);
    for (int l = 0; l < launches; l++)
        k_brick_grow_dev<<<ggrid, BG * BG * BG, 0, c->stream>>>(nb0, nb1, nb2, bmask, seed, buf0, buf1, fs, BG, 0);
    k_grow_finish<<<64, TPB, 0, c->stream>>>(nbr, seed, buf0, buf1, fs, c->blab_buf, box_first, bmask, c->brick_rec, 0, chase && launches < long_schedule ? 1 : 0);
}

static void launch_window_bricks(xb_ctx *c, int *list, int *count, const int *skip) {
    const Grid &g = c->g;
    const int nb0 = c->nbk[0], per_plane = c->nbk[1] * c->nbk[2], nbr = nb0 * per_plane;
    const int w0 = g.wx0 / BRK, wn = g.wlen / BRK, run1 = std::min(wn, nb0 - w0);
    const unsigned grid = (nbr + 16 * TPB - 1) / (16 * TPB);
    k_brick_walk_list<<<grid, TPB, 0, c->stream>>>(nbr, w0 * per_plane, (w0 + run1) * per_plane, c->blab, list, count, skip);
    if (wn > run1) k_brick_walk_list<<<grid, TPB, 0, c->stream>>>(nbr, 0, (wn - run1) * per_plane, c->blab, list, count, skip);
}

static void launch_walk_list(xb_ctx *c, int nb0, int nb1, int nb2, int *walk, const int *bpot, double vac_tol) {
    int bits = 0;
    while ((1 << bits) < std::max(std::max(nb0, nb1), nb2)) bits++;
    const bool linear = bits > XB_MORTON_BITS;
    const unsigned n_codes = linear ? (unsigned)(nb0 * nb1 * nb2) : 1u << (3 * bits);
    k_brick_walk_list_morton<<<(n_codes + 16 * TPB - 1) / (16 * TPB), TPB, 0, c->stream>>>(nb0, nb1, nb2, n_codes, linear ? 1 : 0, c->blab, walk,
                                                                                          c->fs + FS_N_WALK, c->fs + FS_GROW_RETRY, bpot, vac_tol);
}

static bool launch_persistent_trace(xb_ctx *c, bool lean_ok, bool part, const int *box_max, const int *walk, int has_vacuum, int *bres) {
    const Grid &g = c->g;
    const int groups = std::max(1, c->trace_waves / XB_TRACE_WAVES);
    const int lean = lean_ok && light(g).use24 && c->opt.lean ? ((long long)g.wlen * g.nyz <= (1LL << 27) ? 4 : 3) : 0;
    const bool window = table_windowed(c);
    int *ovf = window ? (int *)c->stage : c->ovf_list;
    const int ovf_cap = window ? (int)std::min<size_t>(c->stage_bytes / sizeof(int), 0x7fffffffu) : c->ovf_cap;
    const bool nb = lean && !window && !part && nb_bits_ok(c);
    (nb ? c->stat_nb_traces : lean ? c->stat_lookup_traces : c->stat_generic_traces)++;
    if (lean == 3) c->stat_wide_traces++;
    auto kernel = !lean ? k_ng_trace_g<2, 0>
                : nb ? (lean == 4 ? k_ng_trace_g<2, 4, false, false, true> : k_ng_trace_g<2, 3, false, false, true>)
                : window ? (lean == 4 ? k_ng_trace_g<2, 4, true> : k_ng_trace_g<2, 3, true>)
                : part ? (lean == 4 ? k_ng_trace_g<2, 4, false, true> : k_ng_trace_g<2, 3, false, true>)
                : (lean == 4 ? k_ng_trace_g<2, 4> : k_ng_trace_g<2, 3>);
    kernel<<<groups, XB_WAVE * XB_TRACE_WAVES, 0, c->stream>>>(light(g), c->grad, box_max, c->blab, c->nbk[1], c->nbk[2], walk, c->fs, c->labels,
                                                               c->first, c->max_list, c->max_cap, ovf, ovf_cap, trace_maxsteps(g), has_vacuum,
                                                               8, 1, lean ? bres : nullptr);
    if (window)
        k_ng_trace_list<2><<<512, TPB, 0, c->stream>>>(light(g), c->grad, box_max, c->blab, c->nbk[1], c->nbk[2], ovf, c->fs + FS_N_OVF, c->labels,
                                                       c->first, c->max_list, c->fs + FS_N_MAX, c->max_cap, c->ovf_list, c->counters + CT_N_OVF,
                                                       c->ovf_cap, trace_maxsteps(g), c->rho, c->dist_dev, has_vacuum);
    return lean != 0;
}

enum { BUNI_NONE, BUNI_SCAN, BUNI_MIXED };
static void launch_relabel(xb_ctx *c, int *fs, int n_maxima, bool regions, const int *box_max, int buni, const int *bres) {
    const Grid &g = c->g;
    const GridL gl = light(g);
    const int nb1 = c->nbk[1], nb2 = c->nbk[2], nbr = c->nbk[0] * nb1 * nb2;
    const int *gate = fs ? fs + FS_SORT_OK : nullptr, *n_walk_dev = fs ? fs + FS_N_WALK : nullptr;
    int *ubuf = reinterpret_cast<int *>(c->st);
    if (regions) {
        const int v = g.nz % 4 == 0 ? 4 : 1;
        (v == 4 ? k_relabel_regions_brick<4> : k_relabel_regions_brick<1>)<<<dim3((g.nz / v + 63) / 64, nb1, (g.x1 - g.x0 + RELABEL_X - 1) / RELABEL_X), TPB, 0, c->stream>>>(
            gl, c->labels, c->first, c->blab, nb1, nb2, box_max, fs, gate, fs ? -1 : c->n_boxes);
        if (buni == BUNI_MIXED) k_fill<int><<<(nbr + 4 * TPB - 1) / (4 * TPB), TPB, 0, c->stream>>>(ubuf, XB_MIXED, nbr);
        if (buni != BUNI_NONE && bres)
            k_buni_after_relabel<<<(nbr + 255) / 256, 256, 0, c->stream>>>(nbr, c->blab, box_max, c->first, ubuf, gate, c->walk, n_walk_dev, bres);
        else if (buni != BUNI_NONE) {
            k_buni_after_relabel<<<(nbr + 255) / 256, 256, 0, c->stream>>>(nbr, c->blab, box_max, c->first, ubuf, gate, nullptr, nullptr, nullptr);
            if (fs) k_label_uniform_list<<<2048, TPB, 0, c->stream>>>(gl, c->labels, nb1, nb2, c->walk, 0, n_walk_dev, gate, ubuf);
            else if (c->n_walk)
                k_label_uniform_list<<<(c->n_walk + 3) / 4, TPB, 0, c->stream>>>(gl, c->labels, nb1, nb2, c->walk, c->n_walk, nullptr, nullptr, ubuf);
        }
    } else
        k_relabel<<<nblocks((long long)(g.x1 - g.x0) * g.nyz), TPB, 0, c->stream>>>(g, c->labels, c->first, gate);
    if (fs) k_reset_first<<<8, 256, 0, c->stream>>>(c->first, c->max_aux, 0, fs + FS_N_MAX, gate);
    else if (n_maxima) k_reset_first<<<(unsigned)((n_maxima + 255) / 256), 256, 0, c->stream>>>(c->first, c->max_aux, n_maxima, nullptr, nullptr);
}

static void numbering_done(xb_ctx *c, const int *sorted, int nmax, int64_t *n_maxima) {
    if (sorted) c->maxima_sorted.assign(sorted, sorted + nmax);
    c->label_wire = label_wire_for(nmax);
    c->regions_pending = false;
    c->first_clean = true;
    if (n_maxima) *n_maxima = nmax;
}

extern "C++" template <int K, bool RHO, bool RESUME = false, bool EXPORT = false, bool NB = false>
static void launch_refine_trace(xb_ctx *c, unsigned grid, int block, const int *list, int n_host, const int *n_dev, int *changed, int *escaped,
                                int *ovf_list, int *ovf_count, int ovf_cap, const unsigned char *brec, int *defer_list, int *defer_count,
                                int regions_ok, const int *region_blab, const WalkerIO &wio) {
    k_refine_trace<K, RHO, RESUME, EXPORT, NB><<<grid, block, 0, c->stream>>>(light(c->g), c->grad, c->labels, c->known, list, n_host, n_dev, changed,
                                                                           escaped, ovf_list, ovf_count, ovf_cap, trace_maxsteps(c->g), c->rho,
                                                                           c->dist_dev, brec, defer_list, defer_count, regions_ok, region_blab, wio);
}

static bool lean_retrace_ok(const xb_ctx *c, const unsigned char *brec, bool slab, int regions_ok, const int *region_blab) {
    const Grid &g = c->g;
    return c->opt.lean_retrace && brec && !slab && nb_bits_ok(c) && regions_ok && !region_blab && !table_windowed(c) && g.x0 == 0 && g.x1 == g.nx &&
           g.vlen == g.nx && light(g).use24 && c->N <= (1LL << 27);
}
static void launch_edge_retrace(xb_ctx *c, unsigned grid, int block, const int *list, int n_host, const int *n_dev, int *changed, int *escaped,
                                int *ovf_count, const unsigned char *brec, bool slab, int *defer_list, int *defer_count, int regions_ok,
                                const int *region_blab) {
    if (lean_retrace_ok(c, brec, slab, regions_ok, region_blab)) {
        c->stat_lean_retraces++;
        k_refine_trace_lean<<<grid, block, 0, c->stream>>>(light(c->g), c->grad, c->labels, c->known, list, n_host, n_dev, changed, c->ovf_list, ovf_count,
                                                           c->ovf_cap, trace_maxsteps(c->g), brec);
        return;
    }
    c->stat_generic_retraces++;
    (brec && !slab && nb_bits_ok(c) ? launch_refine_trace<2, false, false, false, true> : launch_refine_trace<2, false>)(
        c, grid, block, list, n_host, n_dev, changed, escaped, c->ovf_list, ovf_count, c->ovf_cap, brec, defer_list, defer_count, regions_ok, region_blab,
        WalkerIO{});
}
static int keep_retrace_overflow(xb_ctx *c, int novf) {
    if (!(c->opt.dbg & XB_DBG_KEEP_RETRACE_OVERFLOW) || novf <= 0) return XB_OK;
    const size_t at = c->dbg_retrace_ovf.size();
    c->dbg_retrace_ovf.resize(at + (size_t)novf);
    HIPCHK(hipMemcpyAsync(c->dbg_retrace_ovf.data() + at, c->ovf_list, (size_t)novf * sizeof(int), hipMemcpyDeviceToHost, c->stream));
    HIPCHK(hipStreamSynchronize(c->stream));
    return XB_OK;
}
```

pybader_amd/csrc/k_edges.h:

```cpp
#pragma once

__device__ __forceinline__ void classify27(const Grid &g, const double *__restrict__ rho,
                                           const int *__restrict__ labels, int x, int y, int z, int v,
                                           bool &is_edge, bool &is_max) {
    const int vol_num = labels[v];
    is_edge = false;
    is_max = true;
    int nb[27];
    int k = 0;
#pragma unroll
    for (int ix = -1; ix < 2; ix++) {
        const int tx = wrapi(x + ix, g.nx);
#pragma unroll
        for (int iy = -1; iy < 2; iy++) {
            const int ty = wrapi(y + iy, g.ny);
#pragma unroll
            for (int iz = -1; iz < 2; iz++) {
                const int tz = wrapi(z + iz, g.nz);
                const int l = lin3(g, tx, ty, tz);
                const int nv = labels[l];
                nb[k++] = (nv == -1) ? -1 : l;
                if (nv != -1 && nv != vol_num) is_edge = true;
            }
        }
    }
    if (!is_edge) return;
    const double max_val = rho[v];
    double nr[27];
#pragma unroll
    for (k = 0; k < 27; k++) nr[k] = rho[nb[k] >= 0 ? nb[k] : v];
#pragma unroll
    for (k = 0; k < 27; k++) is_max &= !(nr[k] > max_val);
}

#define XB_MIXED (-2147483647 - 1)
__global__ __launch_bounds__(256) void k_buni_after_relabel(int nbr, const int *__restrict__ blab, const int *__restrict__ box_max,
                                                            const int *__restrict__ rank, int *__restrict__ buni, const int *gate,
                                                            const int *__restrict__ walk, const int *n_walk, const int *__restrict__ bres) {
    if (gate && !*gate) return;
    const int t = blockIdx.x * blockDim.x + threadIdx.x, nt = gridDim.x * blockDim.x;
    for (int b = t; b < nbr; b += nt) {
        const int l = blab[b];
        if (l > 0) buni[b] = rank[box_max[l - 1]];
    }
    if (!bres) return;
    const int n = *n_walk;
    for (int e = t; e < n; e += nt) {
        const int b = walk[e], r = bres[b];
        buni[b] = r == XB_MIXED ? XB_MIXED : rank[r];
    }
}

__global__ void k_buni3(int nb0, int nb1, int nb2, const int *__restrict__ buni, int *__restrict__ buni3) {
    const int b = blockIdx.x * blockDim.x + threadIdx.x;
    if (b >= nb0 * nb1 * nb2) return;
    const int b0 = b / (nb1 * nb2), b1 = (b / nb2) % nb1, b2 = b % nb2;
    const int l = buni[b];
    bool ok = l != XB_MIXED;
#pragma unroll
    for (int k = 0; k < 27; k++) {
        const int q = buni[(wrap_any(b0 + k / 9 - 1, nb0) * nb1 + wrap_any(b1 + (k / 3) % 3 - 1, nb1)) * nb2 + wrap_any(b2 + k % 3 - 1, nb2)];
        ok &= (q == l);
    }
    buni3[b] = ok ? l : XB_MIXED;
}
__global__ __launch_bounds__(TPB) void k_label_uniform_list(GridL g, const int *__restrict__ labels, int nb1, int nb2,
                                                            const int *__restrict__ walk, int n_walk, const int *n_dev,
                                                            const int *gate, int *__restrict__ buni, int b_off = 0, int nbr = 0) {
    if (gate && !*gate) return;
    const int n = n_dev ? *n_dev : n_walk;
    const int lane = threadIdx.x % XB_WAVE;
    for (int e = blockIdx.x * (TPB / XB_WAVE) + threadIdx.x / XB_WAVE; e < n; e += gridDim.x * (TPB / XB_WAVE)) {
        int b;
        if (walk) b = walk[e];
        else { b = e + b_off; if (b >= nbr) b -= nbr; }
        const int b0 = b / (nb1 * nb2), b1 = (b / nb2) % nb1, b2 = b % nb2;
        int lo = 2147483647, hi = XB_MIXED;
#pragma unroll
        for (int k = 0; k < 8; k++) {
            const int t = lane + k * XB_WAVE;
            const int x = b0 * 8 + t / 64, y = b1 * 8 + (t / 8) % 8, z = b2 * 8 + t % 8;
            if (x < g.nx && y < g.ny && z < g.nz) {
                const int l = labels[(x * g.ny + y) * g.nz + z];
                lo = min(lo, l); hi = max(hi, l);
            }
        }
        for (int o = 32; o > 0; o >>= 1) { lo = min(lo, __shfl_xor(lo, o)); hi = max(hi, __shfl_xor(hi, o)); }
        if (lane == 0) buni[b] = (lo == hi) ? lo : XB_MIXED;
    }
}

__global__ __launch_bounds__(TPB) void k_edge_dilate_list(GridL g, int8_t *known, const int *__restrict__ list, int n_host,
                                                          const int *n_dev) {
    const int n = n_dev ? *n_dev : n_host;
  for (int t = blockIdx.x * TPB + threadIdx.x; t < n; t += gridDim.x * TPB) {
    const int v = list[t];
    const int x = v / g.nyz;
    const int r = v - x * g.nyz;
    const int y = r / g.nz, z = r - y * g.nz;
    int row[9];
#pragma unroll
    for (int j = 0; j < 9; j++) row[j] = (wrapi(x + j / 3 - 1, g.nx) * g.ny + wrapi(y + j % 3 - 1, g.ny)) * g.nz;
    if (z >= 1 && z + 2 < g.nz) {
        unsigned int w[9];
#pragma unroll
        for (int j = 0; j < 9; j++) w[j] = *reinterpret_cast<const unsigned int *>(known + row[j] + z - 1);
#pragma unroll
        for (int j = 0; j < 27; j++)
            if (!((w[j / 3] >> (8 * (j % 3) + 7)) & 1u)) known[row[j / 3] + z - 1 + j % 3] = -1;
    } else {
        int8_t k[27];
#pragma unroll
        for (int j = 0; j < 27; j++) k[j] = known[row[j / 3] + wrapi(z + j % 3 - 1, g.nz)];
#pragma unroll
        for (int j = 0; j < 27; j++)
            if (k[j] >= 0) known[row[j / 3] + wrapi(z + j % 3 - 1, g.nz)] = -1;
    }
  }
}

#define ET_X 4
#define ET_Y 8
#define ET_Z 64
__device__ __forceinline__ void edge_tile(const GridL &g, const double *__restrict__ rho, const int *__restrict__ labels,
                                          int8_t *__restrict__ known, int xa, int nplanes, int *__restrict__ list,
                                          int *list_count, int small, const int *__restrict__ buni,
                                          const GradRec *__restrict__ G, const unsigned char *__restrict__ brick_rec,
                                          int no_vacuum, int tx0, int y0, int z0, int salt = 0) {
    const int tid = (int)threadIdx.x + salt;
    __shared__ int tile[ET_X + 2][ET_Y + 2][ET_Z + 2];
    if (buni) {
        __shared__ int s_lab, s_mixed;
        if (tid == 0) { s_lab = XB_MIXED; s_mixed = 0; }
        __syncthreads();
        const int nb1 = (g.ny + 7) >> 3, nb2 = (g.nz + 7) >> 3;
        int X0 = xa + tx0, X1 = xa + min(tx0 + ET_X, nplanes) - 1;
        if (X0 >= g.nx) X0 -= g.nx;
        if (X1 >= g.nx) X1 -= g.nx;
        const int bxa = X0 >> 3, bxb = X1 >> 3, nbz = min(ET_Z / 8, nb2 - (z0 >> 3));
        if ((int)tid < 2 * nbz) {
            const int bx = (tid & 1) ? bxb : bxa;
            const int l = buni[(bx * nb1 + (y0 >> 3)) * nb2 + (z0 >> 3) + (tid >> 1)];
            if (l == XB_MIXED) s_mixed = 1;
            else {
                const int old = atomicCAS(&s_lab, XB_MIXED, l);
                if (old != XB_MIXED && old != l) s_mixed = 1;
            }
// ... 1491 lines not shown
```

pybader_amd/csrc/k_trace.h:

```cpp
#pragma once

__global__ __launch_bounds__(TPB) void k_fill_certain(GridL g, const int *__restrict__ blab, int nb1, int nb2,
                                                      const int *__restrict__ box_max, int *labels, int *first,
                                                      int *max_list, int *max_count, int max_cap, const int *skip = nullptr) {
    if (skip && *skip) return;
    const int vbeg = g.x0 * g.nyz, vend = g.x1 * g.nyz;
    const int v = vbeg + blockIdx.x * TPB + threadIdx.x;
    const bool in = v < vend;
    int result = -1;
    bool has = false;
    if (in) {
        const int x = v / g.nyz;
        const int r = v - x * g.nyz;
        const int y = r / g.nz, z = r - y * g.nz;
        const int b = blab[((x >> 3) * nb1 + (y >> 3)) * nb2 + (z >> 3)];
        if (b > 0 && labels[v] != -1) {
            result = box_max[b - 1];
            if (result != v && labels[result] == -1) result = -1;
            labels[v] = result;
            has = result >= 0;
        }
    }
    note_maximum_wave(has, result, in ? v : 0, first, max_list, max_count, max_cap);
}
// ... 381 lines not shown
    note_maximum_wave(result >= 0, result, v, first, max_list, max_count, max_cap);
    if (result == -2) {
        const int k = atomicAdd(ovf_count, 1);
        if (k < ovf_cap) ovf_list[k] = v;
    }
    return result;
}
__device__ __forceinline__ void brick_sub_voxel(int b, int sub, int lane, int nb1, int nb2, int &sx, int &sy, int &sz) {
    const int b0 = b / (nb1 * nb2), b1 = (b / nb2) % nb1, b2 = b % nb2;
    sx = b0 * 8 + ((sub >> 2) << 2) + (lane >> 4);
    sy = b1 * 8 + ((sub & 3) << 1) + ((lane >> 3) & 1);
    sz = b2 * 8 + (lane & 7);
}
template <int K, bool WIN>
__global__ __launch_bounds__(TPB) void k_ng_trace(GridL g, const GradRec *__restrict__ G,
                                                  const int *__restrict__ box_max, const int *__restrict__ blab,
                                                  int nb1, int nb2, const int *__restrict__ walk, int n_walk,
                                                  int *labels, int *first,
                                                  int *max_list, int *max_count, int max_cap, int *ovf_list,
                                                  int *ovf_count, int ovf_cap, int maxsteps, int opt,
                                                  const double *__restrict__ rho, const double *__restrict__ gc, int has_vacuum) {
    int blk = blockIdx.x;
    if (opt & 2) {
        const int per = gridDim.x >> 3;
        if (blk < (per << 3)) blk = (blk & 7) * per + (blk >> 3);
    }
    const int wpb = blockDim.x / XB_WAVE;
    const int wave = blk * wpb + threadIdx.x / XB_WAVE;
    const int lane = threadIdx.x % XB_WAVE;
    int sx, sy, sz;
    if (walk) {
        if ((wave >> 3) >= n_walk) return;
        brick_sub_voxel(walk[wave >> 3], wave & 7, lane, nb1, nb2, sx, sy, sz);
        if (sx < g.x0 || sx >= g.x1) return;
    } else if (opt & 1) {
        const int bz_n = (g.nz + 3) >> 2, by_n = (g.ny + 3) >> 2;
        const int bx = wave / (by_n * bz_n);
        const int brem = wave - bx * (by_n * bz_n);
        const int by = brem / bz_n, bz = brem - by * bz_n;
        sx = g.x0 + bx * 4 + (lane >> 4); sy = by * 4 + ((lane >> 2) & 3); sz = bz * 4 + (lane & 3);
    } else {
        const int rz_n = (g.nz + 63) >> 6;
        const int row = wave / rz_n;
        sz = (wave - row * rz_n) * 64 + lane;
        sx = g.x0 + row / g.ny;
        sy = row - (row / g.ny) * g.ny;
    }
    ng_walk_wave<K, WIN>(g, G, box_max, blab, nb1, nb2, walk != nullptr, sx, sy, sz, labels, first, max_list, max_count,
                         max_cap, ovf_list, ovf_count, ovf_cap, maxsteps, rho, gc, has_vacuum != 0);
}
template <int K>
__global__ __launch_bounds__(TPB) void k_ng_trace_list(GridL g, const GradRec *__restrict__ G, const int *__restrict__ box_max,
                                                       const int *__restrict__ blab, int nb1, int nb2,
                                                       const int *__restrict__ vox, const int *n_dev, int *labels, int *first,
                                                       int *max_list, int *max_count, int max_cap, int *ovf_list,
                                                       int *ovf_count, int ovf_cap, int maxsteps,
                                                       const double *__restrict__ rho, const double *__restrict__ gc, int has_vacuum) {
    const int n = *n_dev;
    for (int base = blockIdx.x * TPB; base < n; base += gridDim.x * TPB) {
        const int t = base + threadIdx.x;
        int sx = g.x1, sy = 0, sz = 0;
        if (t < n) {
            const int v = vox[t];
            sx = v / g.nyz;
            const int r = v - sx * g.nyz;
            sy = r / g.nz;
            sz = r - sy * g.nz;
        }
        ng_walk_wave<K, true>(g, G, box_max, blab, nb1, nb2, true, sx, sy, sz, labels, first, max_list, max_count, max_cap,
                              ovf_list, ovf_count, ovf_cap, maxsteps, rho, gc, has_vacuum != 0);
    }
}
__device__ __forceinline__ int xcc_id() {
    int x;
    asm volatile("s_getreg_b32 %0, hwreg(HW_REG_XCC_ID)" : "=s"(x));
    return x & 7;
}

template <int K, int LEAN, bool WINDOW = false, bool PART = false, bool NB = false>
__global__ __launch_bounds__(XB_WAVE * XB_TRACE_WAVES, 8) void k_ng_trace_g(GridL g, const GradRec *__restrict__ G, const int *__restrict__ box_max,
                                                       const int *__restrict__ blab, int nb1, int nb2,
                                                       const int *__restrict__ walk, int *fs, int *labels, int *first,
                                                       int *max_list, int max_cap, int *ovf_list, int ovf_cap, int maxsteps,
                                                       int has_vacuum, int CH, int xcd_split, int *__restrict__ bres = nullptr) {
    __shared__ int s_base, s_next;
    __shared__ int s_w[8], s_mixed;
    constexpr bool CACHE = LEAN >= 3;
    static_assert(!NB || (CACHE && !WINDOW && !PART), "neighbour bits: whole bricks, the whole grid (a cut brick narrower than 5 voxels reaches both sides of an axis)");
    int prev_brick = -1;
#ifdef XB_DEBUG_COUNT
    const long long pr_t0 = clock64();
    long long pr_walk = 0, pr_wait = 0, pr_load = 0;
    int pr_bricks = 0;
    const unsigned long long pr_e0 = wall_clock64();
#endif
    const int n_items = fs[FS_N_WALK] * 8;
    const int per = (((n_items + 7) >> 3) + 7) & ~7;
    const int home = xcd_split ? xcc_id() : (blockIdx.x & 7);
    const int lane = threadIdx.x & (XB_WAVE - 1);
    auto verdict = [&]() {
        if (CACHE && bres && prev_brick >= 0) {
            int r0 = s_mixed ? -1 : s_w[0];
#pragma unroll
            for (int k = 1; k < 8; k++) r0 = (s_w[k] == r0) ? r0 : -1;
            bres[prev_brick] = r0 >= 0 ? r0 : (-2147483647 - 1);
        }
        prev_brick = -1;
    };
    for (int r = 0; r < 8; r++) {
        const int q = (home + r) & 7;
        const int beg = q * per, end = min(beg + per, n_items);
        for (;;) {
#ifdef XB_DEBUG_COUNT
            const long long pr_a = clock64();
#endif
            __syncthreads();
#ifdef XB_DEBUG_COUNT
            pr_wait += clock64() - pr_a;
#endif
            if (threadIdx.x == 0) {
                verdict();
                s_mixed = 0;
                s_base = beg + atomicAdd(&fs[FS_CURSOR0 + q * FS_CURSOR_STRIDE], CH);
                s_next = 0;
            }
            __syncthreads();
            const int base = s_base;
            if (base >= end) break;
            const int stop = min(base + CH, end);
#ifdef XB_DEBUG_COUNT
            const long long pr_b = clock64();
            pr_bricks++;
#endif
            if (CACHE) {
                constexpr int PER = 512 / (XB_WAVE * XB_TRACE_WAVES);
                const int b = walk[base >> 3];
                prev_brick = b;
                const int b0 = b / (nb1 * nb2), b1 = (b / nb2) % nb1, b2 = b % nb2;
                GradRec tmp[PER];
#pragma unroll
                for (int k = 0; k < PER; k++) {
                    const int t = threadIdx.x + k * XB_WAVE * XB_TRACE_WAVES;
                    int cx = b0 * 8 + (t >> 6), cy = b1 * 8 + ((t >> 3) & 7), cz = b2 * 8 + (t & 7);
                    if (PART) { cx = min(cx, g.nx - 1); cy = min(cy, g.ny - 1); cz = min(cz, g.nz - 1); }
                    const int lt = lin24(g, cx, cy, cz);
                    tmp[k] = fetch_rec(G, WINDOW ? rec_slot(g, lt) : lt);
                }
#pragma unroll
                for (int k = 0; k < PER; k++) xb_s_rec[threadIdx.x + k * XB_WAVE * XB_TRACE_WAVES] = tmp[k];
                __syncthreads();
            }
#ifdef XB_DEBUG_COUNT
            pr_load += clock64() - pr_b;
#endif
            for (;;) {
                int i = 0;
                if (lane == 0) i = atomicAdd(&s_next, 1);
                const int item = base + __builtin_amdgcn_readfirstlane(i);
                if (item >= stop) break;
                int sx, sy, sz;
                brick_sub_voxel(walk[item >> 3], item & 7, lane, nb1, nb2, sx, sy, sz);
                if (PART) { sx = min(sx, g.nx - 1); sy = min(sy, g.ny - 1); sz = min(sz, g.nz - 1); }
                if (LEAN) {
#ifdef XB_DEBUG_COUNT
                    const long long pr_c = clock64();
#endif
                    int res;
                    if constexpr (NB) {
                        const int wbrick = walk[item >> 3];
                        res = ng_walk_packed<LEAN == 4>(g, G, box_max, blab, nb1, nb2, (wbrick / (nb1 * nb2)) << 3, ((wbrick / nb2) % nb1) << 3, (wbrick % nb2) << 3,
                                                        sx, sy, sz, labels, first, max_list, &fs[FS_N_MAX], max_cap, ovf_list, &fs[FS_N_OVF], ovf_cap, maxsteps, has_vacuum != 0);
                    } else
                        res = ng_walk_lean<LEAN == 4, CACHE, WINDOW>(g, G, box_max, blab, nb1, nb2, sx, sy, sz, labels, first, max_list, &fs[FS_N_MAX],
                                                                     max_cap, ovf_list, &fs[FS_N_OVF], ovf_cap, maxsteps, has_vacuum != 0);
#ifdef XB_DEBUG_COUNT
                    pr_walk += clock64() - pr_c;
#endif
                    if (CACHE && bres) {
                        volatile int *w = s_w;
                        if (lane == 0) w[item - base] = res;
                        if (w[item - base] != res) *(volatile int *)&s_mixed = 1;
                    }
                }
                else
                    ng_walk_wave<K, false>(g, G, box_max, blab, nb1, nb2, true, sx, sy, sz, labels, first, max_list, &fs[FS_N_MAX],
                                           max_cap, ovf_list, &fs[FS_N_OVF], ovf_cap, maxsteps, nullptr, nullptr, has_vacuum != 0);
            }
        }
    }
#ifdef XB_DEBUG_COUNT
    if (lane == 0 && blockIdx.x < 2048) {
        unsigned long long *o = xb_dbg + 64 + 6 * (blockIdx.x * XB_TRACE_WAVES + (threadIdx.x >> 6));
        o[0] = (unsigned long long)pr_walk; o[1] = (unsigned long long)(clock64() - pr_t0); o[2] = (unsigned long long)pr_wait;
        o[3] = (unsigned long long)pr_load; o[4] = pr_e0; o[5] = (unsigned long long)wall_clock64();
        if (threadIdx.x == 0) xb_dbg[64 + 6 * 8192 + blockIdx.x] = (unsigned long long)pr_bricks;
    }
#endif
    if (CACHE && bres) {
        __syncthreads();
        if (threadIdx.x == 0) verdict();
    }
}

__global__ __launch_bounds__(TPB) void k_list_unfinished(GridL g, const int *__restrict__ walk, const int *n_walk, int nb1, int nb2,
                                                         const int *__restrict__ labels, int *out, int *out_count, int out_cap) {
    __shared__ int s_buf[BlockAppender<2>::CAP], s_n[2];
    BlockAppender<2> app;
    app.init(s_buf, s_n, out, out_count, out_cap);
    const int n = *n_walk;
    for (int e = blockIdx.x; e < n; e += gridDim.x) {
        const int b = walk[e];
        const int b0 = b / (nb1 * nb2), b1 = (b / nb2) % nb1, b2 = b % nb2;
        int v[2];
        int cnt = 0;
#pragma unroll
        for (int k = 0; k < 2; k++) {
            const int t = threadIdx.x + k * TPB;
            const int x = b0 * 8 + (t >> 6), y = b1 * 8 + ((t >> 3) & 7), z = b2 * 8 + (t & 7);
            if (x < g.nx && y < g.ny && z < g.nz) {
                const int l = (x * g.ny + y) * g.nz + z;
                if (labels[l] == -2) v[cnt++] = l;
            }
        }
        app.add(cnt, [&](int k) { return v[k]; });
    }
    app.finish();
}

__global__ void k_path_pack(const int *__restrict__ path, int lmax, const int *__restrict__ off, const int *__restrict__ len,
                            const int *__restrict__ first, int *__restrict__ packed) {
    const int t = blockIdx.x;
    const int *P = path + (size_t)t * lmax;
    if (threadIdx.x == 0) packed[off[t]] = P[0];
    for (int k = first[t] + threadIdx.x; k < len[t]; k += blockDim.x) packed[off[t] + 1 + k - first[t]] = P[k];
}
template <bool SCATTER>
__global__ void k_move_voxels(const int *__restrict__ idx, int n, int *labels, int8_t *known, int *lab_buf, int8_t *kn_buf) {
    const int t = blockIdx.x * blockDim.x + threadIdx.x;
    if (t >= n) return;
    if (SCATTER) { labels[idx[t]] = lab_buf[t]; known[idx[t]] = kn_buf[t]; }
    else { lab_buf[t] = labels[idx[t]]; kn_buf[t] = known[idx[t]]; }
}

__global__ void k_trace_slow(Grid g, const double *__restrict__ rho, int *labels, const int8_t *known_ro,
                             int8_t *known, const int *list, int n, int *path, int lmax, int refine, int *first,
                             int *max_list, int *max_count, int max_cap, int *changed, int *escaped, int *err,
                             int *lens, int has_vacuum = 1, long long sk = 1, long long st = -1, int *retry = nullptr, int *retry_count = nullptr,
                             const int *n_dev = nullptr) {
    const int t = blockIdx.x * blockDim.x + threadIdx.x;
    if (t >= n || (n_dev && t >= *n_dev)) return;
    const int v = list[t];
    if (st < 0) st = lmax;
    int *P0 = path + (size_t)t * st;
#define P(k) P0[(size_t)(k) * sk]
    int np = 0;
    int px = v / g.nyz;
    int r = v - px * g.nyz;
    int py = r / g.nz, pz = r - py * g.nz, lp = v;
    double c = rho[v], dr0 = 0., dr1 = 0., dr2 = 0.;
    const int vol_num = labels[v];
    P(np++) = v;
    int result = -3;
    for (;;) {
        int qx, qy, qz;
        const bool stay = ng_step(rho, g, px, py, pz, lp, c, dr0, dr1, dr2, qx, qy, qz);
        int lq = lin3(g, qx, qy, qz);
        bool on_path = stay;
        for (int k = np - 1; k >= 0 && !on_path; k--) on_path = (P(k) == lq);
        if (on_path) {
            dr0 = dr1 = dr2 = 0.;
            og_step(rho, g, g.dist, px, py, pz, c, qx, qy, qz);
            lq = lin3(g, qx, qy, qz);
            if (qx == px && qy == py && qz == pz) { result = lp; break; }
        }
        if (refine == 1) {
            if (!plane_valid(g, qx)) { known[v] = -6; atomicAdd(escaped, 1); return; }
            if (known_ro[lq] == 2) { result = lq; break; }
        }
        if (np >= lmax) {
            if (refine == 2) {
                lens[t] = -np;
                int fo = np;
// ... 32 lines not shown
```

pybader_amd/csrc/slab_step.h:

```cpp

#define XB_TAB_ROWS 1024
#define XB_TAB_INTS (2 + 2 * XB_TAB_ROWS)
#define XB_SLAB_RANKS_MAX 64
#define XB_XCNT XB_XC_COUNT
__host__ __device__ __forceinline__ size_t walk_part(int cap) { return 16 + (size_t)cap * (sizeof(Walker) + 8); }
static inline int walk_cap_for(const Grid &g) { return (int)std::min<long long>(std::max<long long>(32768, (long long)g.nyz / 8), 1 << 20); }

__global__ void k_slab_flag(const int *fs, int *flags, int rank) { flags[rank] = fs[FS_TIES] != 0; }
__global__ void k_slab_any_flag(const int *flags, int nranks, int *fs) {
    int any = 0;
    for (int r = 0; r < nranks; r++) any |= flags[r];
    fs[FS_TIES] = any;
}
__global__ void k_slab_pack_table(int *tab, const int *__restrict__ max_list, const int *__restrict__ first, int *fs,
                                  const int *slow_count) {
    const int n = fs[FS_N_MAX];
    const bool bad = n > XB_TAB_ROWS || *slow_count > 0 || fs[FS_GROW_RETRY];
    if (threadIdx.x == 0) { tab[0] = bad ? -1 : n; tab[1] = 0; fs[FS_N_REDO] = fs[FS_N_OVF]; fs[FS_N_OVF] = *slow_count; }
    if (bad) return;
    for (int i = threadIdx.x; i < n; i += blockDim.x) {
        const int m = max_list[i];
        tab[2 + 2 * i] = m;
        tab[3 + 2 * i] = first[m];
    }
// ... 223 lines not shown
    Grid &g = c->g;
    const GridL gl = light(g);
    const int nb0 = g.nx / BRK, nb1 = g.ny / BRK, nb2 = g.nz / BRK, nbr = nb0 * nb1 * nb2;
    int *fs = c->fs;
    int *seed = c->list, *bmask = c->list + nbr, *buf0 = c->list + 2 * nbr, *buf1 = c->list + 3 * nbr, *bmaxv = c->list + 4 * nbr,
        *bpot = c->list + 5 * nbr, *reclist = c->list + 6 * nbr;
    int *walk = bmaxv;
    int *box_max = c->boxbuf + BB_REGMAX, *box_first = c->boxbuf + BB_REGFIRST;
    c->box_max_tab = box_max;
    c->labels_zero_pending = false;
    if (int rc = begin_assignment(c, c->counters + CT_N_MAX, CT_INTS(CT_N_MAX, CT_REDO), true)) return rc;
    {
        ScopedTimer t_growth(c, XB_TIMER_MASKS_GROWTH);
        k_slab_any_flag<<<1, 1, 0, c->stream>>>(slab_flags(c), c->slab_nranks, fs);
        launch_region_growth(c, nb0, nb1, nb2, bmask, bmaxv, bpot, seed, buf0, buf1, box_max, box_first, true);
        HIPCHK(hipGetLastError());
    }
    c->blab = c->blab_buf;
    c->walk = walk;
    c->nbk[0] = nb0; c->nbk[1] = nb1; c->nbk[2] = nb2;
    {
        ScopedTimer t_assign(c, XB_TIMER_ASSIGN);
        const int per_plane = nb1 * nb2;
        launch_window_bricks(c, reclist, fs + FS_N_RECL, fs + FS_GROW_RETRY);
        k_brick_walk_list<<<(nbr + 16 * TPB - 1) / (16 * TPB), TPB, 0, c->stream>>>(nbr, (g.x0 / BRK) * per_plane, (g.x1 / BRK) * per_plane, c->blab, walk, fs + FS_N_WALK, fs + FS_GROW_RETRY);
        {
            ScopedTimer t_records(c, XB_TIMER_BRICK_RECORDS);
            launch_brick_records(c, reclist, fs + FS_N_RECL, nbr, nb1, nb2);
        }
        k_note_certain_bricks<<<(nbr + 255) / 256, 256, 0, c->stream>>>(gl, nb0, nb1, nb2, (g.x0 / BRK) * per_plane, (g.x1 / BRK) * per_plane, c->blab,
                                                                      box_max, c->first, c->max_list, fs + FS_N_MAX, c->max_cap, fs + FS_GROW_RETRY);
        c->regions_pending = true;
        {
            ScopedTimer t_trace(c, XB_TIMER_TRACE);
            launch_persistent_trace(c, true, false, box_max, walk, 0, nullptr);
        }
        k_slab_pack_table<<<1, 256, 0, c->stream>>>(slab_tables(c) + (size_t)c->slab_rank * XB_TAB_INTS, c->max_list, c->first, fs, c->counters + CT_N_OVF);
    }
    HIPCHK(hipGetLastError());
    g.main_ties = 0;
    c->slab_stage = 2;
    return XB_OK;
}

int xb_slab_assign_finish(xb_ctx *c, int64_t *n_maxima, int64_t *status) {
    NEED_GRID_RAW("xb_slab_assign_finish");
    if (c->slab_stage != 2) return fail(XB_E_STATE, "xb_slab_assign_finish: call xb_slab_assign_trace first");
    c->slab_stage = 0;
    int *fs = c->fs;
    const int *tabs = slab_tables(c);
    k_slab_merge_min<<<c->slab_nranks, 256, 0, c->stream>>>(tabs, c->first);
    k_slab_merge_list<<<1, 1024, 0, c->stream>>>(tabs, c->slab_nranks, c->max_list, c->max_cap, fs);
    k_number_maxima<<<1, 1024, 0, c->stream>>>(fs, c->first, c->max_list, c->max_cap, c->max_aux);
    launch_relabel(c, fs, 0, true, c->boxbuf + BB_REGMAX, BUNI_MIXED, nullptr);
    HIPCHK(hipGetLastError());
    HIPCHK(hipMemcpyAsync(c->host_ints, fs, FS_COUNT * sizeof(int), hipMemcpyDeviceToHost, c->stream));
    HIPCHK(hipMemcpyAsync(c->host_ints + FS_COUNT, c->max_aux, XB_SORT_MAX * sizeof(int), hipMemcpyDeviceToHost, c->stream));
    HIPCHK(hipStreamSynchronize(c->stream));
    const int *h = c->host_ints;
    if (n_maxima) *n_maxima = 0;
    c->regions_pending = false;
    if (h[FS_GROW_RETRY]) {
        c->grow_kill_launches = 1 << 20;
        c->stat_grow_retries++;
        drop_table(*c);
        if (status) *status = 1;
        return XB_OK;
    }
    if (!h[FS_SORT_OK]) {
        drop_table(*c);
        if (status) *status = 2;
        return XB_OK;
    }
    c->grad_rule = h[FS_TIES] ? 1 : 2;
    c->window_ties = h[FS_TIES] != 0;
    c->n_boxes = h[FS_N_BOXES];
    c->box_voxels = (long long)h[FS_N_CERTAIN] * BRK * BRK * BRK;
    c->n_walk = h[FS_N_WALK];
    if (c->opt.dbg & XB_DBG_SLAB_STATS)
        fprintf(stderr, "[slab %d] bricks traced %d, with records %d, trajectories redone beyond the table window %d, regions %d\n", c->slab_rank,
                h[FS_N_WALK], h[FS_N_RECL], h[FS_N_REDO], h[FS_N_BOXES]);
    numbering_done(c, h + FS_COUNT, h[FS_N_MAX], n_maxima);
    c->buni_valid = true;
    c->buni_halo_safe = true;
    c->regions_labels = true;
    c->table_stage = 2;
    if (status) *status = 0;
    return XB_OK;
}

int xb_slab_refine_pass(xb_ctx *c) {
    NEED_GRID("xb_slab_refine_pass");
    if (int rc = slab_need_xbuf(c)) return rc;
    const Grid &g = c->g;
    if (g.vlen >= g.nx) return fail(XB_E_STATE, "xb_slab_refine_pass: not a slab");
    if (c->slab_nranks < 2) return fail(XB_E_STATE, "xb_slab_refine_pass: call xb_slab_assign_masks first");
    if (int rc = slab_need_wbuf(c)) return rc;
    if (int rc = ensure_grad(c, false, false, false)) return rc;
    bool dilate_owned = false;
    if (int rc = edge_find_launch(c, &dilate_owned)) return rc;
    const GridL gl = light(g);
    if (dilate_owned) {
        ScopedTimer t(c, XB_TIMER_EDGE_FIND);
        k_edge_dilate_list<<<2048, TPB, 0, c->stream>>>(gl, c->known, c->list, 0, c->counters + CT_N_EDGES);
    }
    c->g.main_ties = 0;
    drop_edge_lists(*c); c->buni_valid = false;
    c->walk_n_out = 0; c->walk_n_res = 0; c->walk_out_dev = nullptr;
    c->walk_host.clear(); c->res_host.clear();
    static_assert(CT_OG_MOVED == CT_N_MAX + 4 && CT_N_EDGES == CT_OG_MOVED + 1 && CT_HALO_EDGES == CT_N_EDGES + 1 && CT_TILES_HALO == CT_HALO_EDGES + 17, "two memsets either side of CT_N_EDGES");
    HIPCHK(hipMemsetAsync(c->counters + CT_N_MAX, 0, CT_INTS(CT_N_MAX, CT_OG_MOVED) * sizeof(int), c->stream));
    HIPCHK(hipMemsetAsync(c->counters + CT_HALO_EDGES, 0, CT_INTS(CT_HALO_EDGES, CT_TILES_HALO) * sizeof(int), c->stream));
    {
        ScopedTimer t(c, XB_TIMER_REFINE_TRACE);
        const unsigned char *brec = c->grad_cover == 1 ? c->brick_rec : nullptr;
        const int regions_ok = brec && c->regions_labels && !c->has_vacuum ? 1 : 0;
        const int *slab_regions = slab_regions_of(c);
        int *defer = (int *)c->stage;
        char *part = (char *)c->wbuf[0] + (size_t)c->slab_rank * walk_part(c->wcap);
        HIPCHK(hipMemsetAsync(part, 0, 16, c->stream));
        WalkerIO wio{};
        wio.out = (Walker *)(part + 16); wio.out_count = (int *)part;
        wio.out_cap = walk_send_of(c, c->wcap);
        const unsigned grid = (unsigned)std::min<long long>(nblocks((long long)(g.x1 - g.x0) * g.nyz / 16), 1 << 20);
        launch_refine_trace<2, false, false, true>(c, grid, TPB, c->list, 0, c->counters + CT_N_EDGES, c->counters + CT_CHANGED, c->counters + CT_ESCAPED, c->ovf_list,
                                                   c->counters + CT_N_OVF, c->ovf_cap, brec, defer, c->counters + CT_DEFER, regions_ok, slab_regions, wio);
        launch_refine_trace<2, true>(c, 512, TPB, defer, 0, c->counters + CT_DEFER, c->counters + CT_CHANGED, c->counters + CT_ESCAPED, c->ovf_list, c->counters + CT_N_OVF,
                                     c->ovf_cap, brec, nullptr, nullptr, 0, slab_regions, wio);
    }
    k_slab_walk_clamp<<<1, 1, 0, c->stream>>>((int *)((char *)c->wbuf[0] + (size_t)c->slab_rank * walk_part(c->wcap)), c->counters + CT_WALK_LOST, walk_send_of(c, c->wcap),
                                              walk_results_of(c, c->wcap));
    HIPCHK(hipGetLastError());
    c->slab_stage = 3;
    c->walk_last = -1;
    c->walk_round = 0;
    return XB_OK;
}

int xb_slab_walkers_round(xb_ctx *c, int src, int last) {
    NEED_GRID("xb_slab_walkers_round");
    if (c->slab_stage != 3 || (src != 0 && src != 1)) return fail(XB_E_STATE, "xb_slab_walkers_round: call xb_slab_refine_pass first");
    const Grid &g = c->g;
    const GridL gl = light(g);
    const char *blk = (const char *)c->wbuf[src];
    const dim3 pgrid(8, c->slab_nranks);
    const int cap = c->wcap;
    char *part = (char *)c->wbuf[1 - src] + (size_t)c->slab_rank * walk_part(cap);
    int *n_in = (int *)((char *)c->wk_in + (size_t)cap * sizeof(Walker));
    k_slab_walk_apply<<<pgrid, 256, 0, c->stream>>>(gl, blk, g.x0, g.x1, c->labels, c->known, c->counters + CT_WALK_CHANGED, c->counters + CT_WALK_STUCK, cap,
                                                    last ? nullptr : (int *)part, n_in);
    if (!last) {
        k_slab_walk_collect<<<pgrid, 256, 0, c->stream>>>(gl, blk, g.x0, g.x1, (Walker *)c->wk_in, n_in, c->counters + CT_WALK_LOST, cap);
        k_slab_walk_clamp_in<<<1, 1, 0, c->stream>>>(n_in, c->counters + CT_WALK_ROUNDS, c->walk_round++, cap);
        WalkerIO wio{};
        wio.in = (const Walker *)c->wk_in;
        wio.out = (Walker *)(part + 16); wio.out_count = (int *)part; wio.out_cap = walk_later_of(c, cap);
        wio.res = (int *)(part + 16 + (size_t)cap * sizeof(Walker)); wio.res_count = (int *)part + 1;
        wio.own0 = g.x0; wio.own1 = g.x1;
        const unsigned char *brec = c->grad_cover == 1 ? c->brick_rec : nullptr;
        launch_refine_trace<2, true, true>(c, std::min(cap / TPB, 512), TPB, nullptr, 0, n_in, c->counters + CT_CHANGED, c->counters + CT_ESCAPED, c->ovf_list,
                                           c->counters + CT_N_OVF, c->ovf_cap, brec, nullptr, nullptr, 0, slab_regions_of(c), wio);
        k_slab_walk_clamp<<<1, 1, 0, c->stream>>>((int *)part, c->counters + CT_WALK_LOST, walk_later_of(c, cap), walk_results_of(c, cap));
    } else {
        k_slab_pack_counts<<<1, 1, 0, c->stream>>>(slab_counts(c), c->counters, blk, c->slab_nranks, c->slab_rank, cap);
        c->walk_last = src;
    }
// ... 67 lines not shown
```

Before: 45860 Mvoxels/s.

## Record per-face brick shell labels during trace to prune edge-refine tile lists

During the persistent neargrid trace, each mixed brick now records whether each of its six faces carries a single label, and relabel maps these to ranks. A new k_sweep_need kernel then uses the face labels, not the plain 27-neighbour uniformity test, so a brick next to mixed neighbours whose touching faces match its label is no longer marked for refinement. The aim is to shrink the edge-refine tile list and skip sweeping voxels that cannot change. The cost is extra shared-memory writes and a ballot pass per brick in the trace kernel, another buffer region, and new state that must be invalidated correctly.

```diff
diff --git a/include/bader_hip.h b/include/bader_hip.h
--- a/include/bader_hip.h
+++ b/include/bader_hip.h
@@ -278,6 +278,7 @@
 #define XB_CHECK_BRICK_LOOKUP 128
 #define XB_CHECK_VOXEL_SWEEP 256
 #define XB_CHECK_GENERIC_RETRACE 512
+#define XB_CHECK_BRICK_SHELL 1024
 enum {
     XB_DBG_EC_PASSES = 4,
     XB_DBG_SLAB_STATS = 16,
@@ -294,6 +295,7 @@
 int xb_slow_path_stats(xb_ctx *c, int64_t *assign_total, int64_t *refine_total);
 int xb_deferred_stats(xb_ctx *c, int64_t *refine_total);
 int xb_sweep_stats(xb_ctx *c, int64_t *bit_sweeps, int64_t *voxel_sweeps);
+int xb_tile_list_stats(xb_ctx *c, int64_t *shell_lists, int64_t *brick_lists);
 int xb_retrace_stats(xb_ctx *c, int64_t *lean_launches, int64_t *generic_launches);
 int xb_trace_stats(xb_ctx *c, int64_t *nb_lean_launches, int64_t *lookup_lean_launches, int64_t *generic_launches,
                    int64_t *wide_lean_launches);
diff --git a/pybader_amd/_lib.py b/pybader_amd/_lib.py
--- a/pybader_amd/_lib.py
+++ b/pybader_amd/_lib.py
@@ -22,6 +22,7 @@
 CROSS_CHECK_BRICK_LOOKUP = 128
 CROSS_CHECK_VOXEL_SWEEP = 256
 CROSS_CHECK_GENERIC_RETRACE = 512
+CROSS_CHECK_BRICK_SHELL = 1024
 XB_OPT_DEBUG = 3
 XB_DBG_EC_PASSES, XB_DBG_SLAB_STATS, XB_DBG_STAGE_WAIT, XB_DBG_SHORT_TIERS = 4, 16, 32, 64
 DEBUG_KEEP_RETRACE_OVERFLOW = 128
@@ -212,6 +213,7 @@
     'xb_slow_path_stats': (_int, [_vp, _pi64, _pi64]),
     'xb_deferred_stats': (_int, [_vp, _pi64]),
     'xb_sweep_stats': (_int, [_vp, _pi64, _pi64]),
+    'xb_tile_list_stats': (_int, [_vp, _pi64, _pi64]),
     'xb_edge_list': (_int, [_vp, _vp, _i64, _pi64, _pi64]),
     'xb_retrace_stats': (_int, [_vp, _pi64, _pi64]),
     'xb_trace_stats': (_int, [_vp, _pi64, _pi64, _pi64, _pi64]),
@@ -1386,6 +1388,11 @@
         check(self.lib.xb_sweep_stats(self.h, C.byref(a), C.byref(b)))
         return a.value, b.value
 
+    def tile_list_stats(self):
+        a, b = C.c_int64(), C.c_int64()
+        check(self.lib.xb_tile_list_stats(self.h, C.byref(a), C.byref(b)))
+        return a.value, b.value
+
     def retrace_stats(self):
         a, b = C.c_int64(), C.c_int64()
         check(self.lib.xb_retrace_stats(self.h, C.byref(a), C.byref(b)))
diff --git a/pybader_amd/csrc/bader_hip.hip b/pybader_amd/csrc/bader_hip.hip
--- a/pybader_amd/csrc/bader_hip.hip
+++ b/pybader_amd/csrc/bader_hip.hip
@@ -100,6 +100,7 @@
         int nb_bits = 1;
         int bit_sweep = 1;
         int lean_retrace = 1;
+        int shell_list = 1;
         int io_tiled = 1;
         int dbg = 0;
         int ec_groups = 256;
@@ -141,6 +142,9 @@
     int max_grid[3] = {0, 0, 0};
     std::vector<int> dbg_retrace_ovf;
     int *bres_last = nullptr;
+    int *bshell_last = nullptr;
+    bool shell_marks = false;
+    long long stat_shell_lists = 0, stat_brick_lists = 0;
     int *blab = nullptr;
     int nbk[3] = {0, 0, 0};
     bool brick_max_blanket = false;
@@ -371,7 +375,7 @@
     switch (key) {
     case XB_OPT_REGIONS: c->opt.boxes = (value & XB_REGIONS_BOXES) != 0; c->opt.bricks = (value & XB_REGIONS_BRICKS) != 0; break;
     case XB_OPT_CROSS_CHECK:
-        if (!(ok = value >= 0 && value < 2 * XB_CHECK_GENERIC_RETRACE)) break;
+        if (!(ok = value >= 0 && value < 2 * XB_CHECK_BRICK_SHELL)) break;
         c->opt.mirror = !(value & XB_CHECK_NO_MIRROR);
         c->opt.lean = !(value & XB_CHECK_GENERIC_WALKER);
         c->opt.mask_diag = !(value & XB_CHECK_FULL_TGRAD);
@@ -382,6 +386,7 @@
         c->opt.nb_bits = !(value & XB_CHECK_BRICK_LOOKUP);
         c->opt.bit_sweep = !(value & XB_CHECK_VOXEL_SWEEP);
         c->opt.lean_retrace = !(value & XB_CHECK_GENERIC_RETRACE);
+        c->opt.shell_list = !(value & XB_CHECK_BRICK_SHELL);
         break;
     case XB_OPT_DEBUG: c->opt.dbg = value; break;
     case XB_OPT_EC_GROUPS: if ((ok = value >= 1 && value <= 4096)) c->opt.ec_groups = value; break;
@@ -411,6 +416,12 @@
     if (!c) return fail(XB_E_ARG, "null ctx");
     if (bit_sweeps) *bit_sweeps = c->stat_bit_sweeps;
     if (voxel_sweeps) *voxel_sweeps = c->stat_voxel_sweeps;
+    return XB_OK;
+}
+int xb_tile_list_stats(xb_ctx *c, int64_t *shell_lists, int64_t *brick_lists) {
+    if (!c) return fail(XB_E_ARG, "null ctx");
+    if (shell_lists) *shell_lists = c->stat_shell_lists;
+    if (brick_lists) *brick_lists = c->stat_brick_lists;
     return XB_OK;
 }
 int xb_retrace_stats(xb_ctx *c, int64_t *lean_launches, int64_t *generic_launches) {
diff --git a/pybader_amd/csrc/host_assign.h b/pybader_amd/csrc/host_assign.h
--- a/pybader_amd/csrc/host_assign.h
+++ b/pybader_amd/csrc/host_assign.h
@@ -32,7 +32,10 @@
         if (int rc = ensure_brick_bytes(c, nbr)) return rc;
         ScopedTimer t(c, XB_TIMER_MASKS_GROWTH);
         int *buni = reinterpret_cast<int *>(c->st);
-        if (!c->buni_valid) k_label_uniform_list<<<4096, TPB, 0, c->stream>>>(light(g), c->labels, nb1, nb2, nullptr, nbr, nullptr, nullptr, buni, 0, nbr);
+        if (!c->buni_valid) {
+            k_label_uniform_list<<<4096, TPB, 0, c->stream>>>(light(g), c->labels, nb1, nb2, nullptr, nbr, nullptr, nullptr, buni, 0, nbr);
+            c->shell_marks = false;
+        }
         c->buni_valid = true;
         k_buni3<<<(nbr + 255) / 256, 256, 0, c->stream>>>(nb0, nb1, nb2, buni, buni + nbr);
         k_flag_mixed_bricks<<<(nbr + 255) / 256, 256, 0, c->stream>>>(nbr, buni + nbr, c->brick_rec);
@@ -369,6 +372,7 @@
     HIPCHK(hipGetLastError());
     if (buni != BUNI_NONE) {
         c->buni_valid = true;
+        c->shell_marks = false;
         c->buni_halo_safe = buni == BUNI_MIXED;
     }
     c->regions_labels = regions && !c->has_vacuum && c->regions_neargrid;
@@ -388,7 +392,7 @@
 
 static int fused_numbering_launch(xb_ctx *c) {
     k_number_maxima<<<1, 1024, 0, c->stream>>>(c->fs, c->first, c->max_list, c->max_cap, c->max_aux, c->fs + FS_TOTAL);
-    launch_relabel(c, c->fs, 0, c->regions_pending, c->box_max_tab, BUNI_SCAN, c->bres_last);
+    launch_relabel(c, c->fs, 0, c->regions_pending, c->box_max_tab, BUNI_SCAN, c->bres_last, c->bshell_last);
     HIPCHK(hipGetLastError());
     return XB_OK;
 }
@@ -409,7 +413,7 @@
     k_rank_blocks<<<1, 1024, 0, c->stream>>>(bsum, (int)n_blocks);
     k_rank_assign<<<(nmax + 255) / 256, 256, 0, c->stream>>>(c->first, c->max_list, nmax, bits, wprefix, bsum, c->max_aux, c->fs);
     HIPCHK(hipGetLastError());
-    launch_relabel(c, c->fs, 0, c->regions_pending, c->box_max_tab, BUNI_SCAN, c->bres_last);
+    launch_relabel(c, c->fs, 0, c->regions_pending, c->box_max_tab, BUNI_SCAN, c->bres_last, c->bshell_last);
     HIPCHK(hipGetLastError());
     c->maxima_sorted.resize(nmax);
     HIPCHK(hipMemcpyAsync(c->maxima_sorted.data(), c->max_aux, (size_t)nmax * sizeof(int), hipMemcpyDeviceToHost, c->stream));
@@ -429,6 +433,7 @@
     int *bmaxv = walk;
     int *bpot = c->list + 5 * nbr;
     int *bres = nullptr;
+    int *bshell = nullptr;
     c->box_max_tab = box_max;
     auto stage_done = [&](const char *what) {
         if (c->opt.dbg & XB_DBG_STAGE_WAIT) {
@@ -483,12 +488,14 @@
         {
             ScopedTimer t_trace(c, XB_TIMER_TRACE);
             int *bres_buf = c->has_vacuum ? nullptr : c->list + 6 * nbr;
-            if (launch_persistent_trace(c, true, part, box_max, walk, c->has_vacuum ? 1 : 0, bres_buf)) bres = bres_buf;
+            int *bshell_buf = bres_buf && !part ? c->list + 7 * (size_t)nbr : nullptr;
+            if (launch_persistent_trace(c, true, part, box_max, walk, c->has_vacuum ? 1 : 0, bres_buf, bshell_buf)) { bres = bres_buf; bshell = bshell_buf; }
         }
         HIPCHK(hipGetLastError());
         stage_done("trace");
     }
     c->bres_last = bres;
+    c->bshell_last = bshell;
     if (int rc = fused_numbering_launch(c)) return rc;
     stage_done("numbering + relabel");
     HIPCHK(hipMemcpyAsync(c->host_ints, fs, (FS_TOTAL + XB_SORT_MAX) * sizeof(int), hipMemcpyDeviceToHost, c->stream));
@@ -497,6 +504,7 @@
         c->grad_rule = 2;
         c->regions_pending = false;
         c->buni_valid = !c->has_vacuum;
+        c->shell_marks = c->bshell_last != nullptr;
         c->regions_labels = !c->has_vacuum;
         c->pending_assign = true;
         return XB_OK;
@@ -576,6 +584,7 @@
     }
     numbering_done(c, sorted, nmax, n_maxima);
     c->buni_valid = !c->has_vacuum;
+    c->shell_marks = c->bshell_last != nullptr;
     c->regions_labels = !c->has_vacuum;
     return XB_OK;
 }
@@ -632,6 +641,7 @@
     c->regions_neargrid = false;
     c->walk = walk;
     c->bres_last = nullptr;
+    c->bshell_last = nullptr;
     c->nbk[0] = nb0; c->nbk[1] = nb1; c->nbk[2] = nb2;
     {
         ScopedTimer t_assign(c, XB_TIMER_ASSIGN);
@@ -663,6 +673,7 @@
     }
     numbering_done(c, sorted, nmax, n_maxima);
     c->buni_valid = true;
+    c->shell_marks = false;
     return XB_OK;
 }
 
diff --git a/pybader_amd/csrc/host_refine.h b/pybader_amd/csrc/host_refine.h
--- a/pybader_amd/csrc/host_refine.h
+++ b/pybader_amd/csrc/host_refine.h
@@ -12,14 +12,20 @@
     if (np > run1) HIPCHK(hipMemsetAsync(c->known, 2, (size_t)(np - run1) * g.nyz, c->stream));
     return XB_OK;
 }
-static int *launch_brick_uniformity(xb_ctx *c, const GridL &gl, int b_off, int count, unsigned scan_grid) {
+static int *launch_brick_uniformity(xb_ctx *c, const GridL &gl, int b_off, int count, unsigned scan_grid, bool shell = false) {
     const Grid &g = c->g;
     const int nb0 = (g.nx + 7) / 8, nb1 = (g.ny + 7) / 8, nb2 = (g.nz + 7) / 8, nbr = nb0 * nb1 * nb2;
     int *buni = reinterpret_cast<int *>(c->st);
     if (!c->buni_valid)
         k_label_uniform_list<<<scan_grid, TPB, 0, c->stream>>>(gl, c->labels, nb1, nb2, nullptr, count, nullptr, nullptr, buni, b_off, nbr);
-    k_buni3<<<(nbr + 255) / 256, 256, 0, c->stream>>>(nb0, nb1, nb2, buni, buni + nbr);
+    if (shell && c->buni_valid) k_sweep_need<<<(nbr + 255) / 256, 256, 0, c->stream>>>(nb0, nb1, nb2, buni, buni + 2 * (size_t)nbr, buni + nbr);
+    else k_buni3<<<(nbr + 255) / 256, 256, 0, c->stream>>>(nb0, nb1, nb2, buni, buni + nbr);
     return buni + nbr;
+}
+static bool shell_list_ok(const xb_ctx *c) {
+    const Grid &g = c->g;
+    return c->opt.shell_list && c->buni_valid && c->shell_marks && !c->has_vacuum && g.x0 == 0 && g.x1 == g.nx && g.nx % 8 == 0 &&
+           g.ny % 8 == 0 && g.nz % 8 == 0 && !table_windowed(c) && !small_grid(g);
 }
 
 static bool sweep_bits_ok(const xb_ctx *c, const int *buni) {
@@ -51,6 +57,7 @@
         const GridL gl = light(g);
         const int small = small_grid(g);
         int *buni = nullptr;
+        bool shell = false;
         if ((g.nx % 8 == 0 && g.ny % 8 == 0 && g.nz % 8 == 0) || (whole && g.nx >= 16 && g.ny >= 16 && g.nz >= 16)) {
             const int per_plane = ((g.ny + 7) / 8) * ((g.nz + 7) / 8);
             int b_off = 0, count = ((g.nx + 7) / 8) * per_plane;
@@ -60,11 +67,13 @@
                 count = ((np + 8 + 7 + (p0 % 8)) / 8 + 1) * per_plane;
             }
             if (!c->buni_valid) c->buni_halo_safe = false;
-            buni = launch_brick_uniformity(c, gl, b_off, count, (unsigned)std::min(4096, (count + 3) / 4));
+            shell = whole && shell_list_ok(c) && sweep_bits_ok(c, reinterpret_cast<const int *>(c->st));
+            buni = launch_brick_uniformity(c, gl, b_off, count, (unsigned)std::min(4096, (count + 3) / 4), shell);
         }
         const GradRec *G = c->grad_valid ? c->grad : nullptr;
         const unsigned char *brec = c->grad_valid && c->grad_cover == 1 ? c->brick_rec : nullptr;
         if (whole && sweep_bits_ok(c, buni)) {
+            (shell ? c->stat_shell_lists : c->stat_brick_lists)++;
             const int ntiles = (g.nz / ET_Z) * (g.ny / ET_Y) * (g.nx / ET_X);
             int *tiles = (int *)c->stage;
             HIPCHK(hipMemsetAsync(c->known, 2, (size_t)c->N, c->stream));
@@ -655,8 +664,11 @@
         const int small = small_grid(g);
         int *buni = nullptr;
         int ntiles_listed = 0;
-        if (g.nx >= 16 && g.ny >= 16 && g.nz >= 16)
-            buni = launch_brick_uniformity(c, gl, 0, ((g.nx + 7) / 8) * ((g.ny + 7) / 8) * ((g.nz + 7) / 8), 4096);
+        if (g.nx >= 16 && g.ny >= 16 && g.nz >= 16) {
+            const bool shell = shell_list_ok(c);
+            buni = launch_brick_uniformity(c, gl, 0, ((g.nx + 7) / 8) * ((g.ny + 7) / 8) * ((g.nz + 7) / 8), 4096, shell);
+            (shell ? c->stat_shell_lists : c->stat_brick_lists)++;
+        }
         const unsigned char *brec = (c->grad_valid && c->grad_cover == 1) || late_records ? c->brick_rec : nullptr;
         if (buni) {
             const int ntiles = ((g.nz + ET_Z - 1) / ET_Z) * ((g.ny + ET_Y - 1) / ET_Y) * ((g.nx + ET_X - 1) / ET_X);
diff --git a/pybader_amd/csrc/host_stages.h b/pybader_amd/csrc/host_stages.h
--- a/pybader_amd/csrc/host_stages.h
+++ b/pybader_amd/csrc/host_stages.h
@@ -94,7 +94,8 @@
                                                                                           c->fs + FS_N_WALK, c->fs + FS_GROW_RETRY, bpot, vac_tol);
 }
 
-static bool launch_persistent_trace(xb_ctx *c, bool lean_ok, bool part, const int *box_max, const int *walk, int has_vacuum, int *bres) {
+static bool launch_persistent_trace(xb_ctx *c, bool lean_ok, bool part, const int *box_max, const int *walk, int has_vacuum, int *bres,
+                                    int *bshell = nullptr) {
     const Grid &g = c->g;
     const int groups = std::max(1, c->trace_waves / XB_TRACE_WAVES);
     const int lean = lean_ok && light(g).use24 && c->opt.lean ? ((long long)g.wlen * g.nyz <= (1LL << 27) ? 4 : 3) : 0;
@@ -111,7 +112,7 @@
                 : (lean == 4 ? k_ng_trace_g<2, 4> : k_ng_trace_g<2, 3>);
     kernel<<<groups, XB_WAVE * XB_TRACE_WAVES, 0, c->stream>>>(light(g), c->grad, box_max, c->blab, c->nbk[1], c->nbk[2], walk, c->fs, c->labels,
                                                                c->first, c->max_list, c->max_cap, ovf, ovf_cap, trace_maxsteps(g), has_vacuum,
-                                                               8, 1, lean ? bres : nullptr);
+                                                               8, 1, lean ? bres : nullptr, lean && bres && !part ? bshell : nullptr);
     if (window)
         k_ng_trace_list<2><<<512, TPB, 0, c->stream>>>(light(g), c->grad, box_max, c->blab, c->nbk[1], c->nbk[2], ovf, c->fs + FS_N_OVF, c->labels,
                                                        c->first, c->max_list, c->fs + FS_N_MAX, c->max_cap, c->ovf_list, c->counters + CT_N_OVF,
@@ -120,7 +121,8 @@
 }
 
 enum { BUNI_NONE, BUNI_SCAN, BUNI_MIXED };
-static void launch_relabel(xb_ctx *c, int *fs, int n_maxima, bool regions, const int *box_max, int buni, const int *bres) {
+static void launch_relabel(xb_ctx *c, int *fs, int n_maxima, bool regions, const int *box_max, int buni, const int *bres,
+                           const int *bshell = nullptr) {
     const Grid &g = c->g;
     const GridL gl = light(g);
     const int nb1 = c->nbk[1], nb2 = c->nbk[2], nbr = c->nbk[0] * nb1 * nb2;
@@ -132,7 +134,8 @@
             gl, c->labels, c->first, c->blab, nb1, nb2, box_max, fs, gate, fs ? -1 : c->n_boxes);
         if (buni == BUNI_MIXED) k_fill<int><<<(nbr + 4 * TPB - 1) / (4 * TPB), TPB, 0, c->stream>>>(ubuf, XB_MIXED, nbr);
         if (buni != BUNI_NONE && bres)
-            k_buni_after_relabel<<<(nbr + 255) / 256, 256, 0, c->stream>>>(nbr, c->blab, box_max, c->first, ubuf, gate, c->walk, n_walk_dev, bres);
+            k_buni_after_relabel<<<(nbr + 255) / 256, 256, 0, c->stream>>>(nbr, c->blab, box_max, c->first, ubuf, gate, c->walk, n_walk_dev, bres,
+                                                                           bshell, ubuf + 2 * (size_t)nbr);
         else if (buni != BUNI_NONE) {
             k_buni_after_relabel<<<(nbr + 255) / 256, 256, 0, c->stream>>>(nbr, c->blab, box_max, c->first, ubuf, gate, nullptr, nullptr, nullptr);
             if (fs) k_label_uniform_list<<<2048, TPB, 0, c->stream>>>(gl, c->labels, nb1, nb2, c->walk, 0, n_walk_dev, gate, ubuf);
diff --git a/pybader_amd/csrc/k_edges.h b/pybader_amd/csrc/k_edges.h
--- a/pybader_amd/csrc/k_edges.h
+++ b/pybader_amd/csrc/k_edges.h
@@ -36,7 +36,8 @@
 #define XB_MIXED (-2147483647 - 1)
 __global__ __launch_bounds__(256) void k_buni_after_relabel(int nbr, const int *__restrict__ blab, const int *__restrict__ box_max,
                                                             const int *__restrict__ rank, int *__restrict__ buni, const int *gate,
-                                                            const int *__restrict__ walk, const int *n_walk, const int *__restrict__ bres) {
+                                                            const int *__restrict__ walk, const int *n_walk, const int *__restrict__ bres,
+                                                            const int *__restrict__ bshell = nullptr, int *__restrict__ shell = nullptr) {
     if (gate && !*gate) return;
     const int t = blockIdx.x * blockDim.x + threadIdx.x, nt = gridDim.x * blockDim.x;
     for (int b = t; b < nbr; b += nt) {
@@ -48,6 +49,13 @@
     for (int e = t; e < n; e += nt) {
         const int b = walk[e], r = bres[b];
         buni[b] = r == XB_MIXED ? XB_MIXED : rank[r];
+        if (bshell && r == XB_MIXED) {
+#pragma unroll
+            for (int s = 0; s < 6; s++) {
+                const int q = bshell[b * 6 + s];
+                shell[b * 6 + s] = q == XB_MIXED ? XB_MIXED : rank[q];
+            }
+        }
     }
 }
 
@@ -63,6 +71,40 @@
         ok &= (q == l);
     }
     buni3[b] = ok ? l : XB_MIXED;
+}
+__global__ void k_sweep_need(int nb0, int nb1, int nb2, const int *__restrict__ buni, const int *__restrict__ shell, int *__restrict__ need) {
+    const int b = blockIdx.x * blockDim.x + threadIdx.x;
+    if (b >= nb0 * nb1 * nb2) return;
+    const int b0 = b / (nb1 * nb2), b1 = (b / nb2) % nb1, b2 = b % nb2;
+    const int l = buni[b];
+    int q[27], B[27];
+#pragma unroll
+    for (int k = 0; k < 27; k++) {
+        B[k] = (wrap_any(b0 + k / 9 - 1, nb0) * nb1 + wrap_any(b1 + (k / 3) % 3 - 1, nb1)) * nb2 + wrap_any(b2 + k % 3 - 1, nb2);
+        q[k] = buni[B[k]];
+    }
+    bool same = true, clash = l == XB_MIXED;
+#pragma unroll
+    for (int k = 0; k < 27; k++) {
+        same &= q[k] == l;
+        clash |= q[k] != l && q[k] != XB_MIXED;
+    }
+    bool ok = !clash;
+    if (ok && !same) {
+#pragma unroll
+        for (int k = 0; k < 27; k++) {
+            const int d0 = k / 9 - 1, d1 = (k / 3) % 3 - 1, d2 = k % 3 - 1;
+            if (q[k] == XB_MIXED) {
+                const int *sh = shell + (size_t)B[k] * 6;
+                bool any = false;
+                if (d0) any |= sh[d0 > 0 ? 0 : 1] == l;
+                if (d1) any |= sh[d1 > 0 ? 2 : 3] == l;
+                if (d2) any |= sh[d2 > 0 ? 4 : 5] == l;
+                ok &= any;
+            }
+        }
+    }
+    need[b] = ok ? l : XB_MIXED;
 }
 __global__ __launch_bounds__(TPB) void k_label_uniform_list(GridL g, const int *__restrict__ labels, int nb1, int nb2,
                                                             const int *__restrict__ walk, int n_walk, const int *n_dev,
diff --git a/pybader_amd/csrc/k_trace.h b/pybader_amd/csrc/k_trace.h
--- a/pybader_amd/csrc/k_trace.h
+++ b/pybader_amd/csrc/k_trace.h
@@ -487,9 +487,11 @@
                                                        const int *__restrict__ blab, int nb1, int nb2,
                                                        const int *__restrict__ walk, int *fs, int *labels, int *first,
                                                        int *max_list, int max_cap, int *ovf_list, int ovf_cap, int maxsteps,
-                                                       int has_vacuum, int CH, int xcd_split, int *__restrict__ bres = nullptr) {
+                                                       int has_vacuum, int CH, int xcd_split, int *__restrict__ bres = nullptr,
+                                                       int *__restrict__ bshell = nullptr) {
     __shared__ int s_base, s_next;
     __shared__ int s_w[8], s_mixed;
+    __shared__ int s_res[512];
     constexpr bool CACHE = LEAN >= 3;
     static_assert(!NB || (CACHE && !WINDOW && !PART), "neighbour bits: whole bricks, the whole grid (a cut brick narrower than 5 voxels reaches both sides of an axis)");
     int prev_brick = -1;
@@ -512,6 +514,31 @@
         }
         prev_brick = -1;
     };
+    auto verdict_shell = [&]() {
+        if (CACHE && bshell && prev_brick >= 0) {
+            const int r_lo = s_res[0], r_xh = s_res[4 * 64 + 32], r_yh = s_res[3 * 64], r_zh = s_res[6];
+            const int lz = lane & 7;
+            bool d_xl = false, d_xh = false, d_yl = false, d_yh = false, d_zl = false, d_zh = false;
+#pragma unroll
+            for (int e = 0; e < 8; e++) {
+                const int v = s_res[e * 64 + lane];
+                if (e < 4) d_xl |= lane < 32 && v != r_lo;
+                else d_xh |= lane >= 32 && v != r_xh;
+                if ((e & 3) == 0) d_yl |= v != r_lo;
+                if ((e & 3) == 3) d_yh |= v != r_yh;
+                d_zl |= lz < 2 && v != r_lo;
+                d_zh |= lz >= 6 && v != r_zh;
+            }
+            const bool m_xl = __ballot(d_xl) != 0, m_xh = __ballot(d_xh) != 0, m_yl = __ballot(d_yl) != 0;
+            const bool m_yh = __ballot(d_yh) != 0, m_zl = __ballot(d_zl) != 0, m_zh = __ballot(d_zh) != 0;
+            if (lane < 6) {
+                const bool mixed = lane == 0 ? m_xl : lane == 1 ? m_xh : lane == 2 ? m_yl : lane == 3 ? m_yh : lane == 4 ? m_zl : m_zh;
+                const int r = lane == 1 ? r_xh : lane == 3 ? r_yh : lane == 5 ? r_zh : r_lo;
+                bshell[prev_brick * 6 + lane] = (!mixed && r >= 0) ? r : (-2147483647 - 1);
+            }
+        }
+        if (threadIdx.x != 0) prev_brick = -1;
+    };
     for (int r = 0; r < 8; r++) {
         const int q = (home + r) & 7;
         const int beg = q * per, end = min(beg + per, n_items);
@@ -523,6 +550,7 @@
 #ifdef XB_DEBUG_COUNT
             pr_wait += clock64() - pr_a;
 #endif
+            if (CACHE && bshell && threadIdx.x < XB_WAVE) verdict_shell();
             if (threadIdx.x == 0) {
                 verdict();
                 s_mixed = 0;
@@ -586,6 +614,7 @@
                         if (lane == 0) w[item - base] = res;
                         if (w[item - base] != res) *(volatile int *)&s_mixed = 1;
                     }
+                    if (CACHE && bshell) s_res[((item - base) << 6) + lane] = res;
                 }
                 else
                     ng_walk_wave<K, false>(g, G, box_max, blab, nb1, nb2, true, sx, sy, sz, labels, first, max_list, &fs[FS_N_MAX],
@@ -603,6 +632,7 @@
 #endif
     if (CACHE && bres) {
         __syncthreads();
+        if (bshell && threadIdx.x < XB_WAVE) verdict_shell();
         if (threadIdx.x == 0) verdict();
     }
 }
diff --git a/pybader_amd/csrc/slab_step.h b/pybader_amd/csrc/slab_step.h
--- a/pybader_amd/csrc/slab_step.h
+++ b/pybader_amd/csrc/slab_step.h
@@ -329,6 +329,7 @@
                 h[FS_N_WALK], h[FS_N_RECL], h[FS_N_REDO], h[FS_N_BOXES]);
     numbering_done(c, h + FS_COUNT, h[FS_N_MAX], n_maxima);
     c->buni_valid = true;
+    c->shell_marks = false;
     c->buni_halo_safe = true;
     c->regions_labels = true;
     c->table_stage = 2;
```

Result: no change. 46090 Mvoxels/s, median of 6 (+0.5%).
